# praeclarum/SdfKit

Measured on AMD Instinct MI355X. Metric: Mvoxels/s, 512^3 sphere SDF sample->mesh, higher is better.
Workload: dtype f32 (sampling) / f64 (cell math)

## Files before the change

include/sdfkit_hip.h:

```cpp
#ifndef SDFKIT_HIP_H
#define SDFKIT_HIP_H
#include <stdint.h>
#ifdef __cplusplus
extern "C" {
#endif
#if defined(__GNUC__) || defined(__clang__)
#pragma GCC visibility push(default)
#endif

#define SDFK_ABI_VERSION 6

typedef enum sdfk_status {
    SDFK_OK = 0,
    SDFK_ERR_INVALID = 1,
    SDFK_ERR_NO_DEVICE = 2,
    SDFK_ERR_HIP = 3,
    SDFK_ERR_COMPILE = 4,
    SDFK_ERR_NOMEM = 5,
    SDFK_ERR_UNSUPPORTED = 6
} sdfk_status;

typedef enum sdfk_opcode {
    SDFK_OP_CONST = 0,
    SDFK_OP_X = 1, SDFK_OP_Y = 2, SDFK_OP_Z = 3,
    SDFK_OP_ADD = 4, SDFK_OP_SUB = 5, SDFK_OP_MUL = 6, SDFK_OP_DIV = 7,
    SDFK_OP_NEG = 8, SDFK_OP_ABS = 9, SDFK_OP_SQRT = 10, SDFK_OP_FLOOR = 11,
    SDFK_OP_MIN_SEL = 12,
    SDFK_OP_MAX_SEL = 13,
    SDFK_OP_MIN_IEEE = 14,
    SDFK_OP_MAX_IEEE = 15,
    SDFK_OP_SEL_LT = 16,
    SDFK_OP_VOXEL_NEAREST = 17,
    SDFK_OP_VOXEL_LINEAR = 18,
    SDFK_OP_SIN = 19, SDFK_OP_COS = 20, SDFK_OP_EXP = 21, SDFK_OP_LOG = 22,
    SDFK_OP_ATAN2 = 23
} sdfk_opcode;
#define SDFK_MAX_VOLUMES 8

typedef struct sdfk_op {
    int32_t opcode;
    int32_t a, b, c, d;
    float imm;
} sdfk_op;

typedef struct sdfk_program sdfk_program;
typedef struct sdfk_volume sdfk_volume;
typedef struct sdfk_mesh sdfk_mesh;
typedef struct sdfk_march_job sdfk_march_job;

int sdfk_abi_version(void);
int sdfk_init(int device);
void sdfk_shutdown(void);
int sdfk_set_stream(void* hip_stream);
int sdfk_synchronize(void);
int sdfk_lane_begin(int32_t lane, void* wait_hip_event);
int sdfk_lane_end(int32_t caller_stream_waits);
const char* sdfk_last_error(void);

typedef enum sdfk_option {
    SDFK_OPT_LANES = 1,
    SDFK_OPT_TOKENS = 2,
    SDFK_OPT_GRAPHS = 3,
    SDFK_OPT_COPY_MODE = 4,
    SDFK_OPT_CORNER_EVAL = 5,
    SDFK_OPT_VCOLOR_EVAL = 6,
    SDFK_OPT_DIST_EXCHANGE = 7,
    SDFK_OPT_DIST_LANES = 8,
    SDFK_OPT_HW_QUEUES = 9,
    SDFK_OPT_CODE_CACHE = 10,
    SDFK_OPT_PREFAULT_HUGE = 11,
    SDFK_OPT_DIST_INDEX16 = 12,
    SDFK_OPT_STREAM_PLACEMENT = 13,
    SDFK_OPT_IDLE_LANE = 14,
    SDFK_OPT_IDLE_PROGRAMS = 15,
    SDFK_OPT_ELIDE_VOLUME = 16,
    SDFK_OPT_COLOR_PASSES = 17,
    SDFK_OPT_COUNT_ = 18
} sdfk_option;
int sdfk_set_option(int32_t key, int64_t value);
int sdfk_get_option(int32_t key, int64_t* value);
int sdfk_set_cache_dir(const char* path);

int sdfk_program_create(const sdfk_op* ops, int32_t n_ops, const int32_t out_rgbw[4],
                        int32_t writes_color, sdfk_program** out);
int sdfk_program_check(const sdfk_op* ops, int32_t n_ops, const int32_t out_rgbw[4], int32_t writes_color);
int sdfk_program_create_bound(const sdfk_op* ops, int32_t n_ops, const int32_t out_rgbw[4], int32_t writes_color,
                              const sdfk_volume* const* volumes, int32_t n_volumes, sdfk_program** out);
int sdfk_program_check_bound(const sdfk_op* ops, int32_t n_ops, const int32_t out_rgbw[4], int32_t writes_color, int32_t n_volumes);
const char* sdfk_program_source(const sdfk_program* p);
int sdfk_jit_stats(int64_t* n_compiled, int64_t* n_cache_hits, double* compile_ms_total);
void sdfk_program_destroy(sdfk_program* p);

int sdfk_volume_create(int32_t nx, int32_t ny, int32_t nz, const float min[3], const float max[3],
                       int32_t with_colors, sdfk_volume** out);
int sdfk_volume_create_slab(int32_t nx, int32_t ny, int32_t nz_global, const float min[3],
                            const float max[3], int32_t z0, int32_t nz_local,
                            int32_t with_colors, sdfk_volume** out);
int sdfk_volume_upload(sdfk_volume* v, const float* values, const float* colors3);
int sdfk_volume_download(const sdfk_volume* v, float* values, float* colors3);
int sdfk_volume_device_ptrs(const sdfk_volume* v, void** values, void** colors3);
int sdfk_volume_row_pitch(const sdfk_volume* v, int32_t* pitch_voxels);
void sdfk_volume_free(sdfk_volume* v);

int sdfk_sample(const sdfk_program* p, sdfk_volume* v, int32_t clip_to_bounds);
int sdfk_volume_clip_to_bounds(sdfk_volume* v);

int sdfk_march(const sdfk_volume* v, float iso_value, int32_t step, sdfk_mesh** out);
int sdfk_march_host(const float* values, const float* colors3, int32_t nx, int32_t ny, int32_t nz,
                    const float min[3], const float max[3], float iso_value, int32_t step,
                    sdfk_mesh** out);
int sdfk_sample_march(const sdfk_program* p, const float min[3], const float max[3],
                      int32_t nx, int32_t ny, int32_t nz, int32_t clip_to_bounds,
                      float iso_value, int32_t step, sdfk_mesh** out);
int sdfk_graph_stats(int64_t* jobs, int64_t* launches, int64_t* device_bytes);

int sdfk_march_begin(const sdfk_volume* v, float iso_value, int32_t layer_begin, int32_t layer_end,
                     sdfk_march_job** job, int64_t* n_vertices, int64_t* n_indices);
int sdfk_march_finish(sdfk_march_job* job, int64_t vertex_base, sdfk_mesh** out);
void sdfk_march_job_free(sdfk_march_job* job);

int sdfk_march_slab(const sdfk_volume* v, float iso_value, int32_t layer_begin, int32_t layer_end,
                    int64_t vertex_base, sdfk_mesh** out);
int sdfk_sample_march_slab(const sdfk_program* p, sdfk_volume* slab, int32_t clip_to_bounds, float iso_value,
                           int32_t layer_begin, int32_t layer_end, int64_t vertex_base, sdfk_mesh** out);

#define SDFK_SLAB_HEADER_BYTES 64
int sdfk_mesh_pack(const sdfk_mesh* m, void* dst, int64_t capacity_bytes, int64_t* needed_bytes);
int sdfk_slab_enqueue(const sdfk_program* p, sdfk_volume* slab, int32_t clip_to_bounds, float iso_value,
                      int32_t layer_begin, int32_t layer_end, void* dst, int64_t capacity_bytes,
                      int32_t lane, void* wait_hip_event);
int sdfk_slabs_rebase(void* gathered, int32_t world, int64_t stride_bytes);
int sdfk_slabs_rebase_mirror(void* gathered, int32_t world, int64_t stride_bytes, void* headers_mirror);

#define SDFK_DIST_ID_BYTES 128
int sdfk_dist_unique_id(void* id_out );
int sdfk_dist_init(int32_t world, int32_t rank, const void* id );
typedef int (*sdfk_allgather_fn)(void* ctx, const void* send, void* recv, int64_t bytes_per_rank);
int sdfk_dist_init_host(int32_t world, int32_t rank, sdfk_allgather_fn allgather, void* ctx);
int sdfk_dist_info(int32_t* world, int32_t* rank, int32_t* backend);
void sdfk_dist_shutdown(void);
int sdfk_dist_slab(int32_t nz, int32_t world, int32_t rank, int32_t* layer_begin, int32_t* layer_end, int32_t* z0, int32_t* nz_local);

#if defined(__GNUC__) || defined(__clang__)
#pragma GCC visibility pop
#endif
typedef struct sdfk_dist_session sdfk_dist_session;
#if defined(__GNUC__) || defined(__clang__)
#pragma GCC visibility push(default)
#endif
int sdfk_dist_session_create(const sdfk_program* p, const float min[3], const float max[3], int32_t nx, int32_t ny, int32_t nz,
                             int32_t clip_to_bounds, float iso_value, int32_t depth, sdfk_dist_session** out);
int sdfk_dist_submit(sdfk_dist_session* s);
int sdfk_dist_collect(sdfk_dist_session* s, int64_t* n_vertices_mine, int64_t* n_indices_mine);
int sdfk_dist_counts(const sdfk_dist_session* s, int64_t* counts);
int sdfk_dist_mesh(sdfk_dist_session* s, sdfk_mesh** out);
int sdfk_dist_slab_mesh(sdfk_dist_session* s, sdfk_mesh** out);
int sdfk_dist_gathered(const sdfk_dist_session* s, void** device_ptr, int64_t* stride_bytes);
int sdfk_dist_stats(const sdfk_dist_session* s, int64_t stats[8]);
int sdfk_dist_tune(sdfk_dist_session* s, int32_t steps_per_mode, int64_t* ns_per_config);
int sdfk_dist_enqueue_only(sdfk_dist_session* s);
// ... 205 lines not shown
```

sdfkit_amd/_native.py:

```python
import ctypes as C
import os
import sys

from . import build as _build

_HERE = os.path.dirname(os.path.abspath(__file__))
_lib = None
_inited_device = None


class SdfKitNativeError(RuntimeError):
    def __init__(self, status, message):
        super().__init__(f"sdfkit_hip status {status}: {message}")
        self.status = status


class Op(C.Structure):
    _fields_ = [("opcode", C.c_int32), ("a", C.c_int32), ("b", C.c_int32), ("c", C.c_int32),
                ("d", C.c_int32), ("imm", C.c_float)]


_vp, _i32, _i64, _f = C.c_void_p, C.c_int32, C.c_int64, C.c_float
_fp, _vpp = C.POINTER(C.c_float), C.POINTER(C.c_void_p)
SIGNATURES = {
# ... 89 lines not shown
    "sdfk_points_search": (C.c_int, [_vp, _vp, _i64, _vp, _vp, _vp]),
    "sdfk_points_search_device": (C.c_int, [_vp, _vp, _i64, _vp, _vp, _vp]),
    "sdfk_points_stats": (C.c_int, [_vp, C.POINTER(_i64)]),
    "sdfk_points_knn": (C.c_int, [_vp, _vp, _i64, _i32, _f, _vp, _vp, _vp]),
    "sdfk_points_knn_device": (C.c_int, [_vp, _vp, _i64, _i32, _f, _vp, _vp, _vp]),
    "sdfk_points_radius_count": (C.c_int, [_vp, _vp, _i64, _f, _vp]),
    "sdfk_points_radius_count_device": (C.c_int, [_vp, _vp, _i64, _f, _vp]),
    "sdfk_points_radius_fill": (C.c_int, [_vp, _vp, _i64, _f, _vp, _vp, _vp]),
    "sdfk_points_radius_fill_device": (C.c_int, [_vp, _vp, _i64, _f, _vp, _vp, _vp]),
    "sdfk_points_normals": (C.c_int, [_vp, _i32, _f, _vp, _i64, _vp, _vp]),
    "sdfk_points_normals_device": (C.c_int, [_vp, _i32, _f, _vp, _i64, _vp, _vp]),
    "sdfk_points_to_volume": (C.c_int, [_vp, _vp, _vp, _i32, _f, C.POINTER(_i64)]),
    "sdfk_points_to_volume_device": (C.c_int, [_vp, _vp, _vp, _i32, _f, C.POINTER(_i64)]),
    "sdfk_points_orient_normals": (C.c_int, [_vp, _i32, _f, _i32, _vp, C.POINTER(_i64)]),
    "sdfk_points_orient_normals_device": (C.c_int, [_vp, _i32, _f, _i32, _vp, C.POINTER(_i64)]),
    "sdfk_points_voxel_downsample": (C.c_int, [_vp, _f, _vp, _vp, _vp, _vp, C.POINTER(_i64)]),
    "sdfk_points_voxel_downsample_device": (C.c_int, [_vp, _f, _vp, _vp, _vp, _vp, C.POINTER(_i64)]),
    "sdfk_points_outliers": (C.c_int, [_vp, _i32, _f, _f, _vp, _vp, _vp, _vp, C.POINTER(_i64), C.POINTER(_i64)]),
    "sdfk_points_outliers_device": (C.c_int, [_vp, _i32, _f, _f, _vp, _vp, _vp, _vp, C.POINTER(_i64), C.POINTER(_i64)]),
    "sdfk_points_blend_colors": (C.c_int, [_vp, _vp, _vp, _i64, _i32, _f, _vp, _vp]),
    "sdfk_points_blend_colors_device": (C.c_int, [_vp, _vp, _vp, _i64, _i32, _f, _vp, _vp]),
    "sdfk_points_to_volume_colors": (C.c_int, [_vp, _vp, _vp, _vp, _i32, _f, C.POINTER(_i64)]),
    "sdfk_points_to_volume_colors_device": (C.c_int, [_vp, _vp, _vp, _vp, _i32, _f, C.POINTER(_i64)]),
    "sdfk_points_voxel_downsample_colors": (C.c_int, [_vp, _f, _vp, _vp, _vp, _vp, _vp, _vp, C.POINTER(_i64)]),
    "sdfk_points_voxel_downsample_colors_device": (C.c_int, [_vp, _f, _vp, _vp, _vp, _vp, _vp, _vp, C.POINTER(_i64)]),
    "sdfk_points_cluster": (C.c_int, [_vp, _f, _i32, _vp, _vp, _vp, _vp, C.POINTER(_i64), C.POINTER(_i64)]),
    "sdfk_points_cluster_device": (C.c_int, [_vp, _f, _i32, _vp, _vp, _vp, _vp, C.POINTER(_i64), C.POINTER(_i64)]),
    "sdfk_points_select": (C.c_int, [_vp, _vp, _vp, _i64, _vp, _vp, C.POINTER(_i64)]),
    "sdfk_points_select_device": (C.c_int, [_vp, _vp, _vp, _i64, _vp, _vp, C.POINTER(_i64)]),
    "sdfk_points_free": (None, [_vp]),
    "sdfk_trimesh_create": (C.c_int, [_vp, _i64, _vp, _i64, _vp, _vpp]),
    "sdfk_trimesh_create_device": (C.c_int, [_vp, _i64, _vp, _i64, _vp, _vpp]),
    "sdfk_trimesh_closest": (C.c_int, [_vp, _vp, _i64, _vp, _vp, _vp]),
    "sdfk_trimesh_closest_device": (C.c_int, [_vp, _vp, _i64, _vp, _vp, _vp]),
    "sdfk_trimesh_to_volume": (C.c_int, [_vp, _vp, C.c_float]),
    "sdfk_trimesh_stats": (C.c_int, [_vp, C.POINTER(_i64)]),
    "sdfk_trimesh_sample": (C.c_int, [_vp, _i64, C.c_uint64, _i32, _vp, _vp, _vp, _vp, _vp, C.POINTER(_i64)]),
    "sdfk_trimesh_sample_device": (C.c_int, [_vp, _i64, C.c_uint64, _i32, _vp, _vp, _vp, _vp, _vp, C.POINTER(_i64)]),
    "sdfk_trimesh_components": (C.c_int, [_vp, _vp, _vp, C.POINTER(_i64), C.POINTER(_i64)]),
    "sdfk_trimesh_components_device": (C.c_int, [_vp, _vp, _vp, C.POINTER(_i64), C.POINTER(_i64)]),
    "sdfk_trimesh_topology": (C.c_int, [_vp, C.POINTER(_i64), _vp, _i64]),
    "sdfk_trimesh_topology_device": (C.c_int, [_vp, C.POINTER(_i64), _vp, _i64]),
    "sdfk_trimesh_select": (C.c_int, [_vp, _vp, _vp, _vp, _vp, _vp, _vp, C.POINTER(_i64), C.POINTER(_i64)]),
    "sdfk_trimesh_select_device": (C.c_int, [_vp, _vp, _vp, _vp, _vp, _vp, _vp, C.POINTER(_i64), C.POINTER(_i64)]),
    "sdfk_trimesh_adjacency": (C.c_int, [_vp, _vp, _vp, _vp, C.POINTER(_i64)]),
    "sdfk_trimesh_adjacency_device": (C.c_int, [_vp, _vp, _vp, _vp, C.POINTER(_i64)]),
    "sdfk_trimesh_smooth": (C.c_int, [_vp, _i32, C.c_float, C.c_float, _i32, _vp]),
    "sdfk_trimesh_smooth_device": (C.c_int, [_vp, _i32, C.c_float, C.c_float, _i32, _vp]),
    "sdfk_trimesh_vertex_normals": (C.c_int, [_vp, _vp, _i32, _vp]),
    "sdfk_trimesh_vertex_normals_device": (C.c_int, [_vp, _vp, _i32, _vp]),
    "sdfk_trimesh_weld": (C.c_int, [_vp, C.c_float, _i32, _vp, _vp, _vp, _vp, _vp, _vp, C.POINTER(_i64), C.POINTER(_i64), C.POINTER(_i64)]),
    "sdfk_trimesh_weld_device": (C.c_int, [_vp, C.c_float, _i32, _vp, _vp, _vp, _vp, _vp, _vp, C.POINTER(_i64), C.POINTER(_i64), C.POINTER(_i64)]),
    "sdfk_trimesh_simplify": (C.c_int, [_vp, C.c_float, _i32, _i32, _vp, _vp, _vp, _vp, _vp, _vp, C.POINTER(_i64), C.POINTER(_i64), C.POINTER(_i64)]),
    "sdfk_trimesh_simplify_device": (C.c_int, [_vp, C.c_float, _i32, _i32, _vp, _vp, _vp, _vp, _vp, _vp, C.POINTER(_i64), C.POINTER(_i64), C.POINTER(_i64)]),
    "sdfk_trimesh_raycast": (C.c_int, [_vp, _vp, _vp, _i64, C.c_float, C.c_float, _i32, _vp, _vp, _vp]),
    "sdfk_trimesh_raycast_device": (C.c_int, [_vp, _vp, _vp, _i64, C.c_float, C.c_float, _i32, _vp, _vp, _vp]),
    "sdfk_trimesh_render": (C.c_int, [_vp, _i32, _i32, _fp, _fp, C.c_float, C.c_float, _vp, _vp, _vp]),
    "sdfk_trimesh_render_device": (C.c_int, [_vp, _i32, _i32, _fp, _fp, C.c_float, C.c_float, _vp, _vp, _vp]),
    "sdfk_trimesh_free": (None, [_vp]),
    "sdfk_volume_redistance": (C.c_int, [_vp, _vp, C.c_float, C.c_float, C.POINTER(_i64)]),
    "sdfk_icp_register": (C.c_int, [_vp, _vp, _vp, _i64, _fp, C.POINTER(_i32)]),
    "sdfk_icp_register_device": (C.c_int, [_vp, _vp, _vp, _i64, _fp, C.POINTER(_i32)]),
    "sdfk_icp_register_plane": (C.c_int, [_vp, _vp, _vp, _vp, _i64, _fp, C.POINTER(_i32), C.POINTER(_i64)]),
    "sdfk_icp_register_plane_device": (C.c_int, [_vp, _vp, _vp, _vp, _i64, _fp, C.POINTER(_i32), C.POINTER(_i64)]),
    "sdfk_profile_count": (C.c_int, []),
    "sdfk_profile_get": (C.c_int, [_i32, C.POINTER(C.c_char_p), C.POINTER(C.c_double), C.POINTER(_i64)]),
}


class IcpParams(C.Structure):
    _fields_ = [("max_iterations", C.c_int32), ("good_correspondence_distance", C.c_float),
                ("converged_max_translation", C.c_float), ("converged_max_rotation", C.c_float)]


ALLGATHER_FN = C.CFUNCTYPE(C.c_int, C.c_void_p, C.c_void_p, C.c_void_p, C.c_int64)

OK, ERR_INVALID, ERR_NO_DEVICE, ERR_HIP, ERR_COMPILE, ERR_NOMEM, ERR_UNSUPPORTED = 0, 1, 2, 3, 4, 5, 6

OPT_LANES, OPT_TOKENS, OPT_GRAPHS, OPT_COPY_MODE, OPT_CORNER_EVAL, OPT_VCOLOR_EVAL = 1, 2, 3, 4, 5, 6
OPT_DIST_EXCHANGE, OPT_DIST_LANES, OPT_HW_QUEUES, OPT_CODE_CACHE, OPT_PREFAULT_HUGE, OPT_DIST_INDEX16, OPT_STREAM_PLACEMENT, OPT_IDLE_LANE = 7, 8, 9, 10, 11, 12, 13, 14
OPT_IDLE_PROGRAMS = 15
OPT_ELIDE_VOLUME = 16
OPT_COLOR_PASSES = 17


def library_path():
    return os.environ.get("SDFKIT_HIP_LIBRARY") or os.path.join(_HERE, "libsdfkit_hip.so")


def lib():
    global _lib
    if _lib is None:
        path = library_path()
        if not os.environ.get("SDFKIT_HIP_LIBRARY") and (not os.path.exists(path) or _build.needs_build()):
            try:
                _build.build()
            except Exception as e:
                what = "is missing" if not os.path.exists(path) else "is older than its sources"
                raise RuntimeError(f"libsdfkit_hip.so {what} and could not be built with hipcc: {e}") from e
        if "torch" not in sys.modules and os.environ.get("SDFKIT_NO_TORCH_PRELOAD") != "1":
            try:
                import torch
            except Exception:
                pass
        L = C.CDLL(path)
        for name, (res, args) in SIGNATURES.items():
            fn = getattr(L, name)
            fn.restype = res
            fn.argtypes = args
        _lib = L
    return _lib


def check(status):
    if status != 0:
        raise SdfKitNativeError(status, lib().sdfk_last_error().decode("utf-8", "replace"))


def init(device=None):
    global _inited_device
    if device is None:
        device = int(os.environ.get("LOCAL_RANK", "0"))
    if _inited_device is None:
        check(lib().sdfk_init(device))
        _inited_device = device
    elif _inited_device != device:
        raise RuntimeError(f"sdfkit_hip already initialised on device {_inited_device}")
    return _inited_device


def bind_torch_stream(device=None):
    import torch
    s = torch.cuda.current_stream(device)
    if s.cuda_stream == 0:
        s = torch.cuda.Stream(device)
        torch.cuda.set_stream(s)
    check(lib().sdfk_set_stream(C.c_void_p(s.cuda_stream)))
    return s


class _PinnedBlock:

    def __init__(self, nbytes):
        p = C.c_void_p()
        check(lib().sdfk_host_alloc(int(nbytes), C.byref(p)))
        self.ptr, self.nbytes = p.value, int(nbytes)

    @property
    def __array_interface__(self):
        return {"shape": (self.nbytes,), "typestr": "|u1", "data": (self.ptr, False), "version": 3}

    def __del__(self):
        try:
            if self.ptr and _lib is not None and _inited_device is not None:
                _lib.sdfk_host_free(C.c_void_p(self.ptr))
        except Exception:
            pass
        self.ptr = 0


def pinned_empty(shape, dtype):
    import numpy as np
    dt = np.dtype(dtype)
    n = int(np.prod(shape)) * dt.itemsize
    if n == 0 or os.environ.get("SDFK_PINNED_ARRAYS") == "0":
        return np.empty(shape, dt)
# ... 55 lines not shown
```

sdfkit_amd/build.py:

```python
import os
import re
import subprocess
import sys
from concurrent.futures import ThreadPoolExecutor

HERE = os.path.dirname(os.path.abspath(__file__))
CSRC = os.path.join(HERE, "csrc")
OBJ = os.path.join(CSRC, "_obj")
LIB = os.path.join(HERE, "libsdfkit_hip.so")
SOURCES = ["lib_context.hip", "lib_jit.hip", "lib_volume.hip", "lib_march.hip", "lib_mesh.hip", "lib_dist.hip", "mc_kernels.hip", "lib_points.hip",
           "lib_trimesh.hip", "lib_redistance.hip", "lib_points_knn.hip", "lib_pointcloud.hip", "lib_orient.hip", "lib_points_filter.hip", "lib_trimesh_topology.hip",
           "lib_trimesh_smooth.hip", "lib_trimesh_weld.hip", "lib_points_cluster.hip", "lib_trimesh_simplify.hip", "lib_trimesh_ray.hip"]
HEADERS = ["lib_internal.h", "device_stage.h", "points_grid.h", "points_set.h", "points_knn.h", "points_walk.h", "points_normals.h", "points_orient.h", "points_filter.h", "points_color.h", "points_cluster.h", "device_forest.h", "icp_solve.h", "trimesh_sdf.h", "trimesh_sample.h", "trimesh_handle.h", "trimesh_topology.h", "trimesh_adjacency.h", "trimesh_weld.h", "trimesh_simplify.h", "trimesh_ray.h", "device_sort.h", "redistance.h", "device_scan.h", "device_reduce.h", "mc_kernels.h", "mc_device.h", "mc_decide.h", "mc_params.h", "mc_luts.h", "sample_codegen.h", "vol_pyramid.h", "mathops.h", "dist_rccl.h", "node_local.h",
           "slab_protocol.h", os.path.join("..", "..", "include", "sdfkit_hip.h")]
DEPS = ["exports.map"] + SOURCES + HEADERS
CFLAGS = ["--offload-arch=gfx950", "-O3", "-std=c++17", "-ffp-contract=off", "-fPIC", "-fno-fast-math", "-fvisibility=hidden", "-Wall",
          "-Wno-unused-function"]
EXTRA = os.environ.get("SDFKIT_HIP_CFLAGS", "").split()


def needs_build():
    if not os.path.exists(LIB):
        return True
    t = os.path.getmtime(LIB)
    return any(os.path.getmtime(os.path.join(CSRC, d)) > t for d in DEPS)


def _includes(path, seen):
    if path in seen or not os.path.exists(path):
        return
    seen.add(path)
    with open(path) as f:
        for m in re.finditer(r'^\s*#include\s+"([^"]+)"', f.read(), re.M):
            _includes(os.path.normpath(os.path.join(os.path.dirname(path), m.group(1))), seen)


def _object_for(src, hipcc, verbose, out_dir=None, extra=()):
    out_dir = out_dir or OBJ
    os.makedirs(out_dir, exist_ok=True)
    s = os.path.join(CSRC, src)
    o = os.path.join(out_dir, src.replace(".hip", ".o"))
    deps = set()
    _includes(s, deps)
    if not extra and os.path.exists(o) and all(os.path.getmtime(d) <= os.path.getmtime(o) for d in deps) and \
            os.path.getmtime(os.path.abspath(__file__)) <= os.path.getmtime(o):
        return o
    cmd = [hipcc] + CFLAGS + list(extra) + ["-c", s, "-o", o]
    if verbose:
        print(" ".join(cmd), file=sys.stderr)
    subprocess.check_call(cmd)
    return o


def build(force=False, verbose=False, out=None, extra=()):
    target = out or LIB
    extra = list(extra) + EXTRA
    if not out and not force and not needs_build():
        return LIB
    import fcntl
    with open(target + ".lock", "w") as lock:
        fcntl.flock(lock, fcntl.LOCK_EX)
        if not out and not force and not needs_build():
            return LIB
        hipcc = os.environ.get("HIPCC", "/opt/rocm/bin/hipcc")
        obj_dir = OBJ if not extra else os.path.join(OBJ, "variant_" + re.sub(r"\W+", "_", os.path.basename(target)))
        with ThreadPoolExecutor(max_workers=min(len(SOURCES), os.cpu_count() or 4)) as ex:
            objs = list(ex.map(lambda s: _object_for(s, hipcc, verbose, obj_dir, extra), SOURCES))
        tmp = f"{target}.tmp.{os.getpid()}"
        cmd = [hipcc, "--offload-arch=gfx950", "-shared", "-fPIC", "-Wl,--version-script=" + os.path.join(CSRC, "exports.map"), "-o", tmp] + objs + \
              ["-lhiprtc", "-ldl"]
        if verbose:
            print(" ".join(cmd), file=sys.stderr)
        try:
            subprocess.check_call(cmd)
            os.replace(tmp, target)
        finally:
            if os.path.exists(tmp):
                os.remove(tmp)
    return target


if __name__ == "__main__":
    args = [a for a in sys.argv[1:] if a != "--force"]
    if len(args) >= 1:
        build(force=True, verbose=True, out=os.path.abspath(args[0]), extra=args[1:])
    else:
        build(force="--force" in sys.argv, verbose=True)
```

sdfkit_amd/csrc/lib_context.hip:

```cpp
#include "lib_internal.h"

thread_local std::string t_err;
Config g_cfg;
DeviceState g_state0;
std::atomic<DeviceState*> g_default_state{&g_state0};
std::mutex g_registry_mu;
std::atomic<int> g_contexts_up{0};
std::vector<DeviceState*> g_states{&g_state0};
thread_local DeviceState* t_state = nullptr;
HostArena g_arena;
HostPool g_pool;
std::recursive_mutex g_pool_mu;

int fail(int code, const char* fmt, ...)
{
    char buf[1024];
    va_list ap;
    va_start(ap, fmt);
    vsnprintf(buf, sizeof buf, fmt, ap);
    va_end(ap);
    t_err = buf;
    return code;
}

// ... 358 lines not shown
            g_copy_stats[0] = (int64_t)total;
            g_copy_stats[1] = since(tp0);
            for (auto& p : pieces) { prefault_start(p.dst, p.bytes); g_pool.wait(); }
            g_copy_stats[2] = since(tp0);
            g_copy_stats[4] = 0;
            const int nt = g_pool.size() + 1;
            for (size_t k = 0; k < chunks.size() && e == hipSuccess; k++) {
                const auto tw = std::chrono::steady_clock::now();
                e = hipEventSynchronize(ev[k % kStageSlots]);
                g_copy_stats[4] += since(tw);
                if (e != hipSuccess) break;
                const Chunk c = chunks[k];
                const char* slot = (const char*)g.stage + (k % kStageSlots) * kStageChunk;
                const size_t per = (c.bytes + nt - 1) / nt;
                g_pool.start(nt, [=](int t) {
                    const size_t a = std::min((size_t)t * per, c.bytes), b = std::min(a + per, c.bytes);
                    if (b > a) memcpy(c.dst + a, slot + a, b - a);
                });
                g_pool.wait();
                if (issued < chunks.size()) e = issue(issued++);
            }
        }
        g_copy_stats[3] = since(tp0);
        if (e != hipSuccess) (void)hipStreamSynchronize(g.stream);
        for (auto& x : ev) g.prof_event_pool.push_back(x);
        if (e != hipSuccess) return fail(SDFK_ERR_HIP, "device-to-host copy: %s", hipGetErrorString(e));
        return SDFK_OK;
    }
    size_t k0 = 0;
    while (k0 < pieces.size() && pieces[k0].bytes == 0) k0++;
    prefault_start(pieces[k0].dst, pieces[k0].bytes);
    g_pool.wait();
    for (size_t k = k0; k < pieces.size(); k++) {
        size_t kn = k + 1;
        while (kn < pieces.size() && pieces[kn].bytes == 0) kn++;
        const bool more = kn < pieces.size();
        if (more) prefault_start(pieces[kn].dst, pieces[kn].bytes);
        hipError_t e = hipSuccess;
        if (pieces[k].bytes) {
            e = hipMemcpyAsync(pieces[k].dst, pieces[k].src, pieces[k].bytes, hipMemcpyDeviceToHost, g.stream);
            if (e == hipSuccess) e = hipStreamSynchronize(g.stream);
        }
        if (more) g_pool.wait();
        if (e != hipSuccess) return fail(SDFK_ERR_HIP, "device-to-host copy: %s", hipGetErrorString(e));
        k = kn - 1;
    }
    return SDFK_OK;
}


extern "C" int sdfk_abi_version(void) { return SDFK_ABI_VERSION; }

extern "C" const char* sdfk_last_error(void) { return t_err.c_str(); }

void config_from_env_once();
void config_from_env()
{
    static std::once_flag once;
    std::call_once(once, config_from_env_once);
}
void config_from_env_once()
{
    g_cfg.loaded = true;
    auto geti = [](const char* name, int dflt) { const char* e = getenv(name); return e && *e ? atoi(e) : dflt; };
    auto gets = [](const char* name) { const char* e = getenv(name); return std::string(e ? e : ""); };
    auto ranged = [&](const char* name, int dflt, int lo, int hi) { const int v = geti(name, dflt); return v >= lo && v <= hi ? v : dflt; };
    g_cfg.lanes = ranged("SDFK_LANES", 3, 0, Context::NSIDE);
    g_cfg.tokens = ranged("SDFK_TOKENS", -1, -1, 3);
    g_cfg.graphs = ranged("SDFK_GRAPHS", 1, 0, 2);
    g_cfg.copy_mode = ranged("SDFK_COPY_MODE", 1, 0, 2);
    g_cfg.copy_threads = ranged("SDFK_COPY_THREADS", 0, 0, 256);
    g_cfg.corner_eval = geti("SDFK_NO_CORNER_EVAL", 0) ? 0 : 1;
    g_cfg.vcolor_eval = geti("SDFK_NO_VCOLOR_EVAL", 0) ? 0 : 1;
    g_cfg.dist_exchange = ranged("SDFK_DIST_EXCHANGE", 0, 0, 3);
    g_cfg.dist_lanes = ranged("SDFK_DIST_LANES", 3, 0, 3);
    g_cfg.dist_index16 = geti("SDFK_DIST_INDEX16", 0) ? 1 : 0;
    g_cfg.code_cache = geti("SDFK_NO_CACHE", 0) ? 0 : 1;
    g_cfg.idle_programs = ranged("SDFK_IDLE_PROGRAMS", 32, 0, 1024);
    g_cfg.elide_volume = ranged("SDFK_ELIDE_VOLUME", 2, 0, 2);
    g_cfg.color_passes = ranged("SDFK_COLOR_PASSES", 0, 0, 2);
    g_cfg.prefault_huge = geti("SDFK_PREFAULT_HUGE", 0) ? 1 : 0;
    g_cfg.place_streams = geti("SDFK_STREAM_PLACEMENT", 1) ? 1 : 0;
    g_cfg.idle_lane = geti("SDFK_IDLE_LANE", 1) ? 1 : 0;
    g_cfg.sample_mode = geti("SDFK_SAMPLE_MODE", -1);
    g_cfg.hw_queues = geti("GPU_MAX_HW_QUEUES", 0);
    g_cfg.env_cache_dir = gets("SDFK_CACHE_DIR");
    g_cfg.env_xdg = gets("XDG_CACHE_HOME");
    g_cfg.env_home = gets("HOME");
    g_cfg.jit_flags = gets("SDFK_JIT_FLAGS");
    g_cfg.dump_source = gets("SDFK_DUMP_SOURCE");
    g_cfg.rccl_lib = gets("SDFK_RCCL_LIB");
}


int context_init(int device)
{
    std::lock_guard<std::recursive_mutex> lk(g_mu);
    if (g.inited) return SDFK_OK;
    int n = 0;
    hipError_t e = hipGetDeviceCount(&n);
    if (e != hipSuccess || n <= 0) return fail(SDFK_ERR_NO_DEVICE, "no HIP device: %s", hipGetErrorString(e));
    if (device < 0 || device >= n) return fail(SDFK_ERR_INVALID, "device %d out of range (%d devices)", device, n);
    HIPCHK(hipSetDevice(device));
    hipDeviceProp_t prop;
    HIPCHK(hipGetDeviceProperties(&prop, device));
    if (strncmp(prop.gcnArchName, "gfx950", 6) != 0)
        return fail(SDFK_ERR_NO_DEVICE, "device %d is %s; this library is built for gfx950 (MI355X) only", device, prop.gcnArchName);
    HIPCHK(hipStreamCreateWithFlags(&g.own_stream, hipStreamNonBlocking));
    g.user_stream = g.stream = g.own_stream;
    g.lanes[0].stream = g.own_stream;
    place_streams();
    for (int k = 1; k <= 3 && k <= Context::NSIDE; k++) (void)lane_stream(k);
    g.cur_lane = 0;
    HIPCHK(hipHostMalloc((void**)&g.slots, sizeof(Context::HostSlot) * Context::NSLOTS, hipHostMallocMapped));
    HIPCHK(hipHostGetDevicePointer((void**)&g.slots_dev, g.slots, 0));
    memset(g.slots, 0, sizeof(Context::HostSlot) * Context::NSLOTS);
    g.device = device;
    t_bound_device = device;
    g.inited = true;
    g_contexts_up.fetch_add(1);
    return SDFK_OK;
}

DeviceState* context_claim(int device, bool listed)
{
    std::lock_guard<std::mutex> rl(g_registry_mu);
    DeviceState* st = nullptr;
    if (listed)
        for (DeviceState* q : g_states)
            if (q->listed && q->claimed_device == device) st = q;
    DeviceState* const dflt = g_default_state.load(std::memory_order_relaxed);
    if (!st)
        for (DeviceState* q : g_states)
            if (q->claimed_device < 0 && (listed || q != dflt)) { st = q; break; }
    if (!st) {
        st = new DeviceState();
        g_states.push_back(st);
    }
    st->claimed_device = device;
    st->listed = listed;
    if (listed && (dflt->claimed_device < 0 || !dflt->listed)) g_default_state.store(st, std::memory_order_release);
    return st;
}

void context_unclaim(DeviceState* st)
{
    std::lock_guard<std::mutex> rl(g_registry_mu);
    st->claimed_device = -1;
    st->listed = true;
    if (g_default_state.load(std::memory_order_relaxed) == st)
        for (DeviceState* q : g_states)
            if (q->listed && q->claimed_device >= 0) { g_default_state.store(q, std::memory_order_release); break; }
}


extern "C" int sdfk_init(int device)
{
    config_from_env();
    if (device < 0) return fail(SDFK_ERR_INVALID, "device %d out of range", device);
    DeviceState* prev = t_state;
    DeviceState* st = context_claim(device, true);
    t_state = st;
    const int r = context_init(device);
    if (r) {
        bool inited;
        { std::lock_guard<std::recursive_mutex> lk(st->mu); inited = st->ctx.inited; }
        if (!inited) context_unclaim(st);
        t_state = prev;
    }
    return r;
}

extern "C" void sdfk_shutdown(void)
{
    std::lock_guard<std::recursive_mutex> lk(g_mu);
    bind_thread();
    if (!g.inited) return;
    while (!g.pending.empty()) (void)mesh_resolve(g.pending.front());
    graph_jobs_destroy_all();
    codes_drop_idle();
    if (dist_active()) dist_release();
    (void)hipStreamSynchronize(g.stream);
    prof_drain();
    for (auto e : g.prof_event_pool) (void)hipEventDestroy(e);
    g.prof_event_pool.clear();
    sync_all_lanes();
    for (auto& t : g.tokens) {
        for (auto& e : t.ring) { if (e) (void)hipEventDestroy(e); e = nullptr; }
        t.last = nullptr; t.last_lane = -1; t.next = 0;
    }
    for (auto& lane : g.lanes) {
        for (auto& kv : lane.free_blocks) (void)hipFree(kv.second);
        lane.free_blocks.clear();
        lane.clean_cull_headers.clear();
    }
    for (auto& kv : g.live_blocks) (void)hipFree(kv.first);
    g.live_blocks.clear();
    for (int k = 1; k <= Context::NSIDE; k++) {
        if (g.lane_done[k]) (void)hipEventDestroy(g.lane_done[k]);
        g.lane_done[k] = nullptr;
        bool pooled = false;
        for (const auto& q : g.pool) pooled = pooled || q.s == g.lanes[k].stream;
        if (g.lanes[k].stream && !pooled) (void)hipStreamDestroy(g.lanes[k].stream);
        g.lanes[k].stream = nullptr;
    }
    for (auto& q : g.pool) (void)hipStreamDestroy(q.s);
    g.pool.clear();
    g.foreign_cls.clear();
    g.placed = false;
    g.cls_lane0 = -1;
    g.n_classes = 0;
    if (g.spin_sink) (void)hipFree(g.spin_sink);
    g.spin_sink = nullptr;
    g.cur_lane = 0;
    g.lanes[0].stream = nullptr;
    for (auto& st : g.slot_state) {
        if (st.dropped) (void)hipEventDestroy(st.dropped);
        st = Context::SlotState();
    }
    if (g.stage) (void)hipHostFree(g.stage);
    g.stage = nullptr;
    g.stage_bytes = 0;
    {
        bool last = true;
        {
            std::lock_guard<std::mutex> rl(g_registry_mu);
            for (DeviceState* q : g_states) last = last && (q == &cur_state() || q->claimed_device < 0);
        }
        if (last) {
            std::lock_guard<std::mutex> al(g_arena.mu);
            for (auto& kv : g_arena.free_blocks) (void)hipHostFree(kv.second);
            g_arena.free_blocks.clear();
            g_arena.live.clear();
        }
    }
    if (g.slots) (void)hipHostFree(g.slots);
    g.slots = nullptr;
    g.slots_dev = nullptr;
    g.hints.clear();
    if (g.own_stream) (void)hipStreamDestroy(g.own_stream);
    g.own_stream = nullptr;
    g.stream = g.user_stream = nullptr;
    g.inited = false;
    g_contexts_up.fetch_sub(1);
    g.device = -1;
    context_unclaim(&cur_state());
}

extern "C" int sdfk_set_stream(void* hip_stream)
{
    std::lock_guard<std::recursive_mutex> lk(g_mu);
    if (int r = require_init()) return r;
    HIPCHK(hipStreamSynchronize(g.stream));
    g.user_stream = hip_stream ? (hipStream_t)hip_stream : g.own_stream;
    g.lanes[0].stream = g.user_stream;
    replace_lane0(g.user_stream);
    g.stream = g.lanes[g.cur_lane].stream;
    return SDFK_OK;
}

extern "C" int sdfk_lane_begin(int32_t lane, void* wait_hip_event)
{
    std::lock_guard<std::recursive_mutex> lk(g_mu);
    if (int r = require_init()) return r;
    if (lane < 1 || lane > Context::NSIDE) return fail(SDFK_ERR_INVALID, "sdfk_lane_begin: lane %d out of range 1..%d", lane, Context::NSIDE);
    if (g.cur_lane != 0) return fail(SDFK_ERR_INVALID, "sdfk_lane_begin: already inside a lane section");
    hipStream_t ls = lane_stream(lane);
    if (wait_hip_event) HIPCHK(hipStreamWaitEvent(ls, (hipEvent_t)wait_hip_event, 0));
    g.cur_lane = lane;
    g.stream = ls;
    return SDFK_OK;
}

extern "C" int sdfk_lane_end(int32_t caller_stream_waits)
{
    std::lock_guard<std::recursive_mutex> lk(g_mu);
    if (int r = require_init()) return r;
    if (g.cur_lane == 0) return fail(SDFK_ERR_INVALID, "sdfk_lane_end: not inside a lane section");
    const int lane = g.cur_lane;
    g.cur_lane = 0;
    g.stream = g.lanes[0].stream;
    if (caller_stream_waits) {
        hipEvent_t ev = g.lane_done[lane];
        if (!ev) {
            HIPCHK(hipEventCreateWithFlags(&ev, hipEventDisableTiming));
            g.lane_done[lane] = ev;
        }
        hipError_t e = hipEventRecord(ev, lane_stream(lane));
        if (e == hipSuccess) e = hipStreamWaitEvent(g.lanes[0].stream, ev, 0);
        if (e != hipSuccess) return fail(SDFK_ERR_HIP, "sdfk_lane_end: %s", hipGetErrorString(e));
    }
    return SDFK_OK;
}

extern "C" int sdfk_synchronize(void)
{
    std::lock_guard<std::recursive_mutex> lk(g_mu);
    if (int r = require_init()) return r;
    HIPCHK(hipStreamSynchronize(g.stream));
    sync_all_lanes();
    for (auto& st : g.slot_state) st.drop_pending = false;
    return SDFK_OK;
}

void codes_trim();
extern "C" int sdfk_set_option(int32_t key, int64_t value)
{
    std::lock_guard<std::recursive_mutex> lk(g_mu);
    config_from_env();
    auto in = [&](int64_t lo, int64_t hi) { return value >= lo && value <= hi; };
    switch (key) {
    case SDFK_OPT_LANES: if (!in(0, Context::NSIDE)) break; g_cfg.lanes = (int)value; return SDFK_OK;
    case SDFK_OPT_TOKENS: if (!in(-1, 3)) break; g_cfg.tokens = (int)value; return SDFK_OK;
    case SDFK_OPT_GRAPHS: if (!in(0, 2)) break; g_cfg.graphs = (int)value; return SDFK_OK;
    case SDFK_OPT_COPY_MODE: if (!in(0, 2)) break; g_cfg.copy_mode = (int)value; return SDFK_OK;
    case SDFK_OPT_CORNER_EVAL: if (!in(0, 1)) break; g_cfg.corner_eval = (int)value; return SDFK_OK;
    case SDFK_OPT_VCOLOR_EVAL: if (!in(0, 1)) break; g_cfg.vcolor_eval = (int)value; return SDFK_OK;
    case SDFK_OPT_DIST_EXCHANGE: if (!in(0, 3)) break; g_cfg.dist_exchange = (int)value; return SDFK_OK;
    case SDFK_OPT_DIST_LANES: if (!in(0, 3)) break; g_cfg.dist_lanes = (int)value; return SDFK_OK;
    case SDFK_OPT_DIST_INDEX16: if (!in(0, 1)) break; g_cfg.dist_index16 = (int)value; return SDFK_OK;
    case SDFK_OPT_STREAM_PLACEMENT: if (!in(0, 1)) break; g_cfg.place_streams = (int)value; return SDFK_OK;
    case SDFK_OPT_IDLE_LANE: if (!in(0, 1)) break; g_cfg.idle_lane = (int)value; return SDFK_OK;
    case SDFK_OPT_CODE_CACHE: if (!in(0, 1)) break; g_cfg.code_cache = (int)value; return SDFK_OK;
    case SDFK_OPT_IDLE_PROGRAMS: if (!in(0, 1024)) break; g_cfg.idle_programs = (int)value; codes_trim(); return SDFK_OK;
    case SDFK_OPT_ELIDE_VOLUME: if (!in(0, 2)) break; g_cfg.elide_volume = (int)value; return SDFK_OK;
    case SDFK_OPT_COLOR_PASSES: if (!in(0, 2)) break; g_cfg.color_passes = (int)value; return SDFK_OK;
    case SDFK_OPT_PREFAULT_HUGE: if (!in(0, 1)) break; g_cfg.prefault_huge = (int)value; return SDFK_OK;
    case SDFK_OPT_HW_QUEUES: return fail(SDFK_ERR_INVALID, "SDFK_OPT_HW_QUEUES is read-only");
    default: return fail(SDFK_ERR_INVALID, "sdfk_set_option: unknown option %d", key);
    }
    return fail(SDFK_ERR_INVALID, "sdfk_set_option(%d): value %lld out of range", key, (long long)value);
}

extern "C" int sdfk_get_option(int32_t key, int64_t* value)
{
    std::lock_guard<std::recursive_mutex> lk(g_mu);
    if (!value) return fail(SDFK_ERR_INVALID, "sdfk_get_option: null argument");
    config_from_env();
    switch (key) {
    case SDFK_OPT_LANES: *value = g_cfg.lanes; break;
    case SDFK_OPT_TOKENS: *value = g_cfg.tokens; break;
    case SDFK_OPT_GRAPHS: *value = g_cfg.graphs; break;
    case SDFK_OPT_COPY_MODE: *value = g_cfg.copy_mode; break;
    case SDFK_OPT_CORNER_EVAL: *value = g_cfg.corner_eval; break;
    case SDFK_OPT_VCOLOR_EVAL: *value = g_cfg.vcolor_eval; break;
    case SDFK_OPT_DIST_EXCHANGE: *value = g_cfg.dist_exchange; break;
    case SDFK_OPT_DIST_LANES: *value = g_cfg.dist_lanes; break;
    case SDFK_OPT_DIST_INDEX16: *value = g_cfg.dist_index16; break;
    case SDFK_OPT_STREAM_PLACEMENT: *value = g_cfg.place_streams; break;
    case SDFK_OPT_IDLE_LANE: *value = g_cfg.idle_lane; break;
    case SDFK_OPT_CODE_CACHE: *value = g_cfg.code_cache; break;
    case SDFK_OPT_IDLE_PROGRAMS: *value = g_cfg.idle_programs; break;
    case SDFK_OPT_ELIDE_VOLUME: *value = g_cfg.elide_volume; break;
    case SDFK_OPT_COLOR_PASSES: *value = g_cfg.color_passes; break;
    case SDFK_OPT_PREFAULT_HUGE: *value = g_cfg.prefault_huge; break;
    case SDFK_OPT_HW_QUEUES: *value = g_cfg.hw_queues; break;
    default: return fail(SDFK_ERR_INVALID, "sdfk_get_option: unknown option %d", key);
    }
    return SDFK_OK;
}

extern "C" int sdfk_set_cache_dir(const char* path)
{
    std::lock_guard<std::recursive_mutex> lk(g_mu);
    config_from_env();
    g_cfg.cache_dir_set = path != nullptr;
    g_cfg.cache_dir = path ? path : "";
    return SDFK_OK;
}

extern "C" int sdfk_host_alloc(int64_t n_bytes, void** out)
{
    if (!out || n_bytes < 0) return fail(SDFK_ERR_INVALID, "sdfk_host_alloc: bad argument");
    *out = nullptr;
    if (g_contexts_up.load() <= 0) {
        std::lock_guard<std::recursive_mutex> lk(g_mu);
        if (int r = require_init()) return r;
    }
    const size_t c = size_class((size_t)std::max<int64_t>(n_bytes, 1));
    std::lock_guard<std::mutex> al(g_arena.mu);
    auto it = g_arena.free_blocks.upper_bound(c);
    void* p = nullptr;
    if (it != g_arena.free_blocks.begin() && std::prev(it)->first == c) {
        --it;
        p = it->second;
        g_arena.free_blocks.erase(it);
    } else if (hipHostMalloc(&p, c, hipHostMallocPortable) != hipSuccess) {
        (void)hipGetLastError();
        for (auto& kv : g_arena.free_blocks) (void)hipHostFree(kv.second);
        g_arena.free_blocks.clear();
        if (hipHostMalloc(&p, c, hipHostMallocPortable) != hipSuccess) { (void)hipGetLastError(); return fail(SDFK_ERR_NOMEM, "hipHostMalloc(%zu) failed", c); }
    }
    g_arena.live[p] = c;
    *out = p;
    return SDFK_OK;
}

extern "C" void sdfk_host_free(void* p)
{
    if (!p) return;
    std::lock_guard<std::mutex> al(g_arena.mu);
    auto it = g_arena.live.find(p);
    if (it == g_arena.live.end()) return;
    g_arena.free_blocks.emplace(it->second, p);
    g_arena.live.erase(it);
}

extern "C" int sdfk_stream_placement(int32_t out[8])
{
    std::lock_guard<std::recursive_mutex> lk(g_mu);
    if (!out) return fail(SDFK_ERR_INVALID, "sdfk_stream_placement: null argument");
    if (int r = require_init()) return r;
    out[0] = g.placed && !g.pool.empty() ? 1 : 0;
    out[1] = g.n_classes;
    out[2] = g.cls_lane0;
    for (int k = 1; k <= 4; k++) {
        out[2 + k] = -1;
        for (const auto& q : g.pool)
            if (k <= Context::NSIDE && q.s == g.lanes[k].stream) out[2 + k] = q.cls;
    }
    out[7] = -1;
    for (const auto& q : g.pool)
        if (q.user == 100) out[7] = q.cls;
    return SDFK_OK;
}

extern "C" int sdfk_copy_stats(int64_t stats[5])
{
    std::lock_guard<std::recursive_mutex> lk(g_mu);
    if (!stats) return fail(SDFK_ERR_INVALID, "sdfk_copy_stats: null argument");
    memcpy(stats, g_copy_stats, sizeof g_copy_stats);
    return SDFK_OK;
}
// ... 53 lines not shown
```

sdfkit_amd/csrc/lib_internal.h:

```cpp
#pragma once
#include <hip/hip_runtime.h>
#include <hip/hiprtc.h>

#include <fcntl.h>
#include <sys/mman.h>
#include <sys/stat.h>
#include <unistd.h>

#include <algorithm>
#include <atomic>
#include <cerrno>
#include <chrono>
#include <cmath>
#include <condition_variable>
#include <cstdarg>
#include <cstdio>
#include <cstring>
#include <deque>
#include <functional>
#include <map>
#include <memory>
#include <mutex>
#include <string>
#include <thread>
#include <unordered_map>
#include <vector>

#include <rccl/rccl.h>

#include "../../include/sdfkit_hip.h"
#include "mc_kernels.h"
#include "sample_codegen.h"

using namespace sdfk;

extern thread_local std::string t_err;
static constexpr int kSampleRpw = 2;


struct Config {
    bool loaded = false;
    int lanes = 3;
    int tokens = -1;
    int graphs = 1;
    int copy_mode = 1;
    int corner_eval = 1;
    int vcolor_eval = 1;
    int dist_exchange = 0;
    int dist_lanes = 3;
    int dist_index16 = 0;
    int code_cache = 1;
    int idle_programs = 32;
    int color_passes = 0;
    int elide_volume = 2;
    int prefault_huge = 0;
    int place_streams = 1;
    int idle_lane = 1;
    int copy_threads = 0;
    int sample_mode = -1;
    int hw_queues = 0;
    std::string cache_dir;
    bool cache_dir_set = false;
    std::string jit_flags;
    std::string dump_source;
    std::string env_cache_dir, env_xdg, env_home, rccl_lib;
};
extern Config g_cfg;

int fail(int code, const char* fmt, ...);
#define HIPCHK(expr)                                                                              \
    do {                                                                                          \
        hipError_t e_ = (expr);                                                                   \
        if (e_ != hipSuccess) return fail(SDFK_ERR_HIP, "%s: %s (%s:%d)", #expr, hipGetErrorString(e_), __FILE__, __LINE__); \
    } while (0)

struct sdfk_mesh;
struct sdfk_volume;
struct ProgCode;



struct ProfSpan { int name_id; hipEvent_t a, b; };

struct Context {
    bool inited = false;
    int device = -1;
    hipStream_t stream = nullptr;
    hipStream_t user_stream = nullptr;
    hipStream_t own_stream = nullptr;
    static constexpr int NSIDE = 4;
    struct Lane { hipStream_t stream = nullptr; std::multimap<size_t, void*> free_blocks; std::vector<uint32_t*> clean_cull_headers; };
    Lane lanes[1 + NSIDE];
    struct Placed { hipStream_t s; int cls; int user; };
    std::vector<Placed> pool;
    std::map<hipStream_t, int> foreign_cls;
    int cls_lane0 = -1, n_classes = 0;
    bool placed = false;
    int* spin_sink = nullptr;
    hipEvent_t lane_done[1 + NSIDE] = {};
    int cur_lane = 0;
    int side_lanes = 2;
    int next_side = 0;
    struct Token { hipEvent_t ring[8] = {}; int next = 0; hipEvent_t last = nullptr; int last_lane = -1; };
    Token tokens[2];
    int token_mask = 0;
    struct Block { size_t size; int lane; };
    std::map<void*, Block> live_blocks;
    bool prof_on = false;
    bool sampler_only = false;
    std::vector<std::string> prof_names;
    std::vector<double> prof_ms;
    std::vector<int64_t> prof_n;
    std::vector<ProfSpan> prof_pending;
    std::vector<hipEvent_t> prof_event_pool;
    struct HostSlot { McCounters c; float bounds[8]; };
    static constexpr int NSLOTS = 64;
    HostSlot* slots = nullptr;
    HostSlot* slots_dev = nullptr;
    int slot_next = 0;
    struct SlotState { bool busy = false; bool drop_pending = false; hipEvent_t dropped = nullptr; };
    SlotState slot_state[NSLOTS];
    void* stage = nullptr;
    size_t stage_bytes = 0;
    struct Hint { uint32_t n_active, nv, ni; };
    std::map<uint64_t, Hint> hints;
    std::deque<sdfk_mesh*> pending;
    static constexpr size_t MAX_PENDING = 6;
    std::vector<struct GraphJob*> graph_jobs;
    uint64_t graph_clock = 0;
    size_t graph_bytes = 0;
    int64_t graph_launches = 0;
    std::map<uint64_t, uint32_t> graph_sightings;
};

struct RcclApi {
    void* handle = nullptr;
    ncclResult_t (*GetUniqueId)(ncclUniqueId*) = nullptr;
    ncclResult_t (*CommInitRank)(ncclComm_t*, int, ncclUniqueId, int) = nullptr;
    ncclResult_t (*CommDestroy)(ncclComm_t) = nullptr;
    ncclResult_t (*AllGather)(const void*, void*, size_t, ncclDataType_t, ncclComm_t, hipStream_t) = nullptr;
    ncclResult_t (*Send)(const void*, size_t, ncclDataType_t, int, ncclComm_t, hipStream_t) = nullptr;
    ncclResult_t (*Recv)(void*, size_t, ncclDataType_t, int, ncclComm_t, hipStream_t) = nullptr;
    ncclResult_t (*GroupStart)() = nullptr;
    ncclResult_t (*GroupEnd)() = nullptr;
    const char* (*GetErrorString)(ncclResult_t) = nullptr;
};

struct DistContext {
    int backend = 0;
    int world = 1, rank = 0;
    RcclApi nccl;
    ncclComm_t comm = nullptr;
    hipStream_t stream = nullptr;
    bool stream_owned = false;
    sdfk_allgather_fn host_fn = nullptr;
    void* host_ctx = nullptr;
    int64_t* agree_dev = nullptr;
    int64_t* agree_host = nullptr;
    char* stage = nullptr;
    int64_t stage_stride = 0;
    int sessions = 0;
    int (*consensus_fn)(void* ctx, int mine) = nullptr;
    void* consensus_ctx = nullptr;
};

struct DeviceState {
    Context ctx;
    std::recursive_mutex mu;
    DistContext dist;
    std::unordered_map<std::string, ProgCode*> codes;
    uint64_t code_clock = 0;
    int graph_build_failures = 0;
    int claimed_device = -1;
    bool listed = true;
// ... 102 lines not shown
        if (threads.empty())
            for (int i = 0; i < size(); i++) threads.emplace_back([this] { worker(); });
        fn = std::move(f);
        ntasks = n;
        next = 0;
        generation++;
        cv_work.notify_all();
    }
    void wait()
    {
        std::unique_lock<std::mutex> lk(mu);
        while (next < ntasks) {
            const int t = next++;
            running++;
            lk.unlock();
            fn(t);
            lk.lock();
            running--;
        }
        cv_done.wait(lk, [&] { return running == 0; });
        ntasks = 0;
    }
    ~HostPool()
    {
        {
            std::unique_lock<std::mutex> lk(mu);
            stopping = true;
            cv_work.notify_all();
        }
        for (auto& t : threads) t.join();
    }
};

extern HostPool g_pool;
extern std::recursive_mutex g_pool_mu;

struct CopyPiece { const void* src; void* dst; size_t bytes; };

constexpr int kTwoPassMaxOps = 24;
constexpr size_t kTwoPassMinVoxels = size_t(1) << 21;
enum ProgKernel { PK_BITS = 0, PK_BITS_FLAT = 1, PK_SIGNS = 2, PK_BITS_CLIP = 3, PK_BITS_CLIP_FLAT = 4, PK_VCOLORS = 5, PK_CORNERS = 6, PK_RAYMARCH = 7,
                  PK_SIGNS_FLAT = 8, PK_CULL = 9, PK_EVAL_BLOCKS = 10, PK_POINTS = 11,
                  PK_BITS_NC = 12, PK_BITS_NC_FLAT = 13, PK_BITS_NC_CLIP = 14, PK_BITS_NC_CLIP_FLAT = 15, PK_COLORS = 16, PK_COUNT = 17 };
inline bool pk_is_sampler(int k) { return k <= PK_BITS_CLIP_FLAT || k == PK_SIGNS_FLAT || k == PK_CULL || k == PK_EVAL_BLOCKS || (k >= PK_BITS_NC && k <= PK_BITS_NC_CLIP_FLAT); }

struct ProgCode {
    std::string source;
    std::vector<hipModule_t> modules;
    hipFunction_t fn[PK_COUNT] = {};
    int refs = 0;
    uint64_t last_use = 0;
};

struct sdfk_program {
    ProgCode* code = nullptr;
    std::vector<float> params;
    int writes_color = 0;
    int n_ops = 0;
    int refs = 1;
    bool orphaned = false;
    bool no_elide = false;
    void* vol_mem = nullptr;
    DeviceState* owner = nullptr;
    std::vector<uint64_t> kbuf;
    void* kargs() const { return kbuf.empty() ? (void*)const_cast<float*>(params.data()) : (void*)const_cast<uint64_t*>(kbuf.data()); }
};

struct sdfk_volume {
    DeviceState* owner = &cur_state();
    int nx = 0, ny = 0, nz = 0;
    int nz_global = 0, z0 = 0;
    float gmin[3], gmax[3];
    float* values = nullptr;
    float* colors = nullptr;
    bool elided = false, elided_colors = false;
    uint32_t* cull_list = nullptr;
    uint32_t* cull_header = nullptr;
    mutable bool cull_header_clean = false;
    int cull_header_lane = 0;
    uint64_t* bits = nullptr;
    uint8_t* bits8 = nullptr;
    float bits_iso = 0.0f;
    bool bits_valid = false;
    sdfk_program* sampled_by = nullptr;
    SampleArgs sampled_args;
    int pitch() const { return (nz + 3) & ~3; }
    size_t nvox() const { return (size_t)nx * ny * nz; }
    size_t nalloc() const { return (size_t)nx * ny * pitch(); }
    int nxw() const { return (nx + 63) / 64; }
    int nx8() const { return (nx + 7) / 8; }
    int pitch8() const { return (nz + 3) & ~3; }
    size_t nbitwords() const { return (size_t)nz * ny * nxw() + 8; }
};

struct sdfk_mesh {
    DeviceState* owner = &cur_state();
    int64_t nv = 0, ni = 0;
    float* vertices = nullptr;
    float* colors = nullptr;
    float* normals = nullptr;
    int32_t* triangles = nullptr;
    float* bounds = nullptr;
    float h_min[3] = {0, 0, 0}, h_max[3] = {0, 0, 0};
    bool bounds_valid = false;
    int64_t n_active = 0, n_case13 = 0;
    size_t cap_v = 0, cap_i = 0;
    sdfk_march_job* pending = nullptr;
    hipEvent_t done = nullptr;
    const sdfk_volume* src = nullptr;
    bool owns_src = false;
    float iso = 0.0f;
    int step = 1, layer_begin = 0, layer_end = 0;
    int64_t vertex_base = 0;
    uint64_t key = 0;
    int status = 0;
    std::string error;
    bool has_colors = true;
    bool colors_valid = true;
    bool external = false;
    struct GraphJob* graph_job = nullptr;
    bool borrowed = false;
    void* slab_header = nullptr;
    int lane = 0;
    bool used_on_main = false;
};

struct sdfk_march_job {
    McParams P;
    McCounters c;
    std::vector<void*> owned;
    sdfk_volume* sub = nullptr;
    int gnx, gny, gnz;
    float gmin[3], gmax[3];
    bool finished = false;
    bool empty = false;
    bool have_bits = false;
    uint8_t* bits8 = nullptr;
    sdfk_program* eval_prog = nullptr;
    SampleArgs eval_args;
    bool colors_elided = false;
    int slot = -1;
    int lane = 0;
    bool* cull_clean = nullptr;
    float* bounds_partial = nullptr;
    int bounds_blocks = 0;
    uint2* vdesc = nullptr;
    size_t vdesc_cap = 0;
    size_t rec_first = 0;
};


int mesh_resolve(sdfk_mesh* m);
void graph_job_retire(sdfk_mesh* m, bool too_small);
void graph_jobs_destroy_all();
void graph_jobs_forget_volume(const sdfk_volume* v);
void graph_jobs_forget_program(const sdfk_program* p);
void dist_release();
bool dist_active();
void resolve_dependents(const sdfk_volume* v);
void free_mesh_buffers(sdfk_mesh* m);
void drop_source(sdfk_mesh* m);
void job_release(sdfk_march_job* j, bool kernels_may_be_queued = false);
void program_release(sdfk_program* p);
void volume_values_changed(sdfk_volume* v);
void codes_drop_idle();



struct GraphJob;
struct PostCompact { char* out; int64_t out_capacity; unsigned long long* ticket; };

void codes_trim();
size_t size_class(size_t n);
int dev_alloc(void** p, size_t n);
void dev_free(void* p);
hipStream_t lane_stream(int k);
void phase_token_wait(int kind);
void phase_token_pass(int kind);
void sync_all_lanes();
double chains_us(hipStream_t a, hipStream_t b);
int stream_class(hipStream_t s, const std::vector<hipStream_t>& reps, double serial_us);
void assign_placed_streams();
void place_streams();
void replace_lane0(hipStream_t s0);
hipStream_t placed_exchange_stream();
int prof_name_id(const char* name);
hipEvent_t prof_event();
void prof_drain();
int require_init();
void bind_thread();
int grid_for(size_t work_items, int per_block = 256, int max_blocks = 256 * 8);
void prefault_start(void* p, size_t n);
int stage_reserve();
int copy_to_host(const std::vector<CopyPiece>& pieces, const std::function<void()>& beside = nullptr);
void config_from_env();
void config_from_env_once();
int context_init(int device);
DeviceState* context_claim(int device, bool listed);
void context_unclaim(DeviceState* st);
uint64_t fnv1a64(const std::string& s, uint64_t h);
std::string cache_dir();
bool cache_load(const std::string& path, const std::string& key, std::vector<char>& code);
void cache_store(const std::string& path, const std::string& key, const std::vector<char>& code);
int compile_source(const std::string& src, unsigned mask, std::vector<char>& code, bool use_cache, bool* from_cache = nullptr,
                          bool refresh = false);
void code_unload(ProgCode* c);
ProgCode* code_acquire(std::string&& src);
void code_release(ProgCode* c);
int generate_source(const sdfk_op* ops, int32_t n_ops, const int32_t out_rgbw[4], int32_t writes_color, std::string& src,
                           std::vector<float>* params = nullptr, int n_volumes = 0);
int program_fn(const sdfk_program* cp, int k, hipFunction_t* fn);
int job_volume_create(const sdfk_program* p, int nx, int ny, int nz, const float mn[3], const float mx[3], float iso, sdfk_volume** out);
int volume_materialize(sdfk_volume* v);
dim3 transpose_grid(int nz, int ny, int nxw);
dim3 flat_grid(size_t plane, int nx8);
void grid_constants(const sdfk_volume* v, float d[3], float m[3], float* outside);
int sample_impl(const sdfk_program* p, sdfk_volume* v, int32_t clip_to_bounds, float iso_hint);
int acquire_slot();
int alloc_records(sdfk_march_job* j, size_t c);
// ... 31 lines not shown
```

sdfkit_amd/csrc/lib_march.hip:

```cpp
#include "lib_internal.h"



template <typename T>
int job_alloc(sdfk_march_job* j, T** p, size_t count)
{
    void* q = nullptr;
    if (int r = dev_alloc(&q, count * sizeof(T))) return r;
    j->owned.push_back(q);
    *p = (T*)q;
    return SDFK_OK;
}

int acquire_slot()
{
    for (int pass = 0; pass < 2; pass++) {
        int oldest = -1;
        for (int i = 0; i < Context::NSLOTS; i++) {
            const int s = (g.slot_next + i) % Context::NSLOTS;
            Context::SlotState& st = g.slot_state[s];
            if (st.busy) continue;
            if (st.drop_pending) {
                if (hipEventQuery(st.dropped) != hipSuccess) { if (oldest < 0) oldest = s; continue; }
                st.drop_pending = false;
            }
            st.busy = true;
            g.slot_next = (s + 1) % Context::NSLOTS;
            memset(&g.slots[s], 0, sizeof(Context::HostSlot));
            return s;
        }
        if (oldest < 0) break;
        (void)hipEventSynchronize(g.slot_state[oldest].dropped);
    }
    return -1;
}

void job_release(sdfk_march_job* j, bool kernels_may_be_queued)
{
    if (j->slot >= 0) {
        Context::SlotState& st = g.slot_state[j->slot];
        st.busy = false;
        st.drop_pending = false;
        if (kernels_may_be_queued) {
            hipError_t e = hipSuccess;
            if (!st.dropped) e = hipEventCreateWithFlags(&st.dropped, hipEventDisableTiming);
            if (e == hipSuccess) e = hipEventRecord(st.dropped, lane_stream(j->lane));
            if (e == hipSuccess) st.drop_pending = true;
            else (void)hipStreamSynchronize(lane_stream(j->lane));
        }
        j->slot = -1;
    }
    for (void* p : j->owned) dev_free(p);
    j->owned.clear();
    if (j->eval_prog) program_release(j->eval_prog);
    j->eval_prog = nullptr;
    if (j->sub) {
        dev_free(j->sub->values);
        dev_free(j->sub->colors);
        delete j->sub;
        j->sub = nullptr;
    }
}

#ifndef SDFK_COMPACT_MASKS
#define SDFK_COMPACT_MASKS 1
#endif
#ifndef SDFK_COMPACT_STRIDED
#define SDFK_COMPACT_STRIDED 1
#endif

int alloc_records(sdfk_march_job* j, size_t c)
{
    McParams& P = j->P;
    for (size_t k = j->rec_first; k < j->owned.size(); k++) dev_free(j->owned[k]);
    j->owned.resize(j->rec_first);
    j->bounds_partial = nullptr;
    j->vdesc = nullptr;
    j->vdesc_cap = 0;
    int rr = 0;
    rr = rr ? rr : job_alloc(j, &P.rec_xy, c);
    rr = rr ? rr : job_alloc(j, &P.rec_z, c);
    rr = rr ? rr : job_alloc(j, &P.rec_info, c);
    rr = rr ? rr : job_alloc(j, &P.rec_own, c);
    rr = rr ? rr : job_alloc(j, &P.rec_pre, c);
    rr = rr ? rr : job_alloc(j, &P.rec_corners, c * 8);
    rr = rr ? rr : job_alloc(j, &P.rec_vid, (c / MC_CHUNK + 1) * (size_t)MC_VSTRIDE);
    rr = rr ? rr : job_alloc(j, &P.chunkslots, c / MC_CHUNK + 2);
    rr = rr ? rr : job_alloc(j, &P.chunktot, c / MC_CHUNK + 2);
    rr = rr ? rr : job_alloc(j, &P.chunkpre, c / MC_CHUNK + 2);
    rr = rr ? rr : job_alloc(j, &P.chunkdead, c / MC_CHUNK + 2);
    rr = rr ? rr : job_alloc(j, &P.chunkwin, c / MC_CHUNK + 2);
    rr = rr ? rr : job_alloc(j, &P.chunkwin2, c / MC_CHUNK + 2);
    P.cap_active = (uint32_t)c;
    P.chunkscan = c / MC_CHUNK + 1 > MC_SCAN_CHUNKS ? 1 : 0;
    return rr;
}

int launch_classify(sdfk_march_job* j, bool publish)
{
    McParams& P = j->P;
    if (!j->have_bits) {
        uint64_t* bits = const_cast<uint64_t*>(P.bits);
        ProfScope ps("k_signbits");
        const int nx8 = (P.nx + 7) / 8, pitch8 = P.nzp;
        if ((P.nz % 256) != 0 || P.ny > 65535 || nx8 > 65535)
            hipLaunchKernelGGL(k_signbits8<true>, flat_grid((size_t)P.ny * pitch8, nx8), dim3(256), 0, g.stream,
                               P.values, j->bits8, P.nx, P.ny, P.nz, nx8, pitch8, P.iso);
        else
            hipLaunchKernelGGL(k_signbits8<false>, dim3((P.nz + 255) / 256, P.ny, nx8), dim3(256), 0, g.stream, P.values, j->bits8, P.nx, P.ny,
                               P.nz, nx8, pitch8, P.iso);
        hipLaunchKernelGGL(k_bits_transpose, transpose_grid(P.nz, P.ny, P.nxw), dim3(256), 0, g.stream, j->bits8, bits,
                           nx8, P.ny, P.nz, P.nxw, pitch8);
        HIPCHK(hipGetLastError());
        j->have_bits = true;
    }
    {
        ProfScope ps("k_compact");
        const int nwg = ((P.lay_list_end - P.lay_count_begin + K2_LPB - 1) / K2_LPB) * P.bpl;
        hipLaunchKernelGGL(k_compact<false>, dim3(nwg), dim3(256), 0, g.stream, P);
        HIPCHK(hipGetLastError());
        if (P.zero_cull && j->cull_clean && nwg > 0) *j->cull_clean = true;
        if (P.blockpre) hipLaunchKernelGGL(k_blockscan, dim3(1), dim3(1024), 0, g.stream, P);
        if (SDFK_COMPACT_STRIDED && K2_LPB == 1)
            if (P.segmask) hipLaunchKernelGGL(k_compact_write<true>, dim3((P.lay_list_end - P.lay_count_begin) * P.bpl), dim3(256), 0, g.stream, P);
            else hipLaunchKernelGGL(k_compact_write<false>, dim3((P.lay_list_end - P.lay_count_begin) * P.bpl), dim3(256), 0, g.stream, P);
        else
            hipLaunchKernelGGL(k_compact<true>, dim3(nwg), dim3(256), 0, g.stream, P);
        HIPCHK(hipGetLastError());
    }
    const int nchunks = (int)((P.cap_active + MC_CHUNK - 1u) / MC_CHUNK);
    if (j->eval_prog) {
        hipFunction_t fn_corners = nullptr;
        if (int r = program_fn(j->eval_prog, PK_CORNERS, &fn_corners)) return r;
        ProfScope ps("sdfk_corners_eval");
        const unsigned* n_active = &P.counters->n_active;
        void* params[] = {&j->eval_args, &P.rec_xy, &P.rec_z, &P.rec_corners, &n_active, &P.cap_active, &P.xbits, j->eval_prog->kargs()};
        HIPCHK(hipModuleLaunchKernel(fn_corners, (unsigned)std::min(nchunks, 256 * 8), 1, 1, 256, 1, 1, 0,
                                     g.stream, params, nullptr));
    } else {
        ProfScope ps("k_gather_corners");
        hipLaunchKernelGGL(k_gather_corners, dim3(std::min(nchunks, 256 * 8)), dim3(256), 0, g.stream, P);
        HIPCHK(hipGetLastError());
    }
    {
        ProfScope ps("k_resolve");
        constexpr int cap = 256 * 12;
        hipLaunchKernelGGL(k_resolve, dim3(std::min(nchunks, cap)), dim3(256), 0, g.stream, P);
        if (P.chunkscan) hipLaunchKernelGGL(k_chunkscan, dim3(1), dim3(1024), 0, g.stream, P);
        if (publish) hipLaunchKernelGGL(k_publish, dim3(1), dim3(256), 0, g.stream, P);
        HIPCHK(hipGetLastError());
    }
    return SDFK_OK;
}

int wait_counters(sdfk_march_job* j)
{
    HIPCHK(hipStreamSynchronize(g.stream));
    j->c = g.slots[j->slot].c;
    return SDFK_OK;
}

int setup_job(const sdfk_volume* v, float iso, int step, int layer_begin, int layer_end, size_t cap_records,
              sdfk_march_job** out)
{
    *out = nullptr;
    if (step < 1) return fail(SDFK_ERR_INVALID, "step must be >= 1");
    const bool slab = (v->z0 != 0 || v->nz != v->nz_global);
    if (step != 1 && (slab || layer_begin != 0)) return fail(SDFK_ERR_UNSUPPORTED, "slab meshing supports step == 1 only");
    sdfk_march_job* j = new sdfk_march_job();
    j->gnx = v->nx; j->gny = v->ny; j->gnz = v->nz_global;
    memcpy(j->gmin, v->gmin, sizeof j->gmin);
    memcpy(j->gmax, v->gmax, sizeof j->gmax);
    j->lane = g.cur_lane;
    j->slot = acquire_slot();
    if (j->slot < 0) { delete j; return fail(SDFK_ERR_NOMEM, "more than %d marching-cubes jobs are alive", Context::NSLOTS); }
    const sdfk_volume* w = v;
    if (step > 1) {
        sdfk_volume* s = new sdfk_volume(*v);
        s->nx = (v->nx - 1) / step + 1; s->ny = (v->ny - 1) / step + 1; s->nz = (v->nz - 1) / step + 1;
        s->nz_global = s->nz;
        s->values = nullptr; s->colors = nullptr; s->bits = nullptr; s->bits8 = nullptr; s->bits_valid = false; s->sampled_by = nullptr;
        j->sub = s;
        int r = dev_alloc((void**)&s->values, s->nalloc() * sizeof(float));
        if (!r && v->colors) r = dev_alloc((void**)&s->colors, s->nalloc() * 3 * sizeof(float));
        if (r) { job_release(j); delete j; return r; }
        ProfScope ps("k_subsample");
        hipLaunchKernelGGL(k_subsample, dim3(grid_for(s->nvox())), dim3(256), 0, g.stream, v->values, v->colors,
                           s->values, s->colors, v->nx, v->ny, v->pitch(), s->nx, s->ny, s->nz, s->pitch(), step);
        w = s;
        layer_end = s->nz - 1;
    }
    McParams& P = j->P;
    memset(&P, 0, sizeof P);
    P.values = w->values; P.colors = w->colors;
    j->colors_elided = w->elided && w->elided_colors;
    if (w->elided && w->cull_header && w->cull_header_lane == g.cur_lane) { P.zero_cull = w->cull_header; j->cull_clean = &w->cull_header_clean; }
    if (w->elided && (step != 1 || !w->sampled_by || !g_cfg.corner_eval || (w->elided_colors && !g_cfg.vcolor_eval) || !w->bits_valid || w->bits_iso != iso)) {
        job_release(j); delete j;
        return fail(SDFK_ERR_INVALID, "internal: a volume without storage can only be meshed by the program that sampled it (step 1, same iso)");
    }
    P.nx = w->nx; P.ny = w->ny; P.nz = w->nz;
    P.nzp = w->pitch();
    {
        auto bits = [](int n) { int b = 0; while ((1 << b) < n) b++; return b; };
        const int bx = bits(w->nx), by = bits(w->ny);
        P.xbits = by > 16 ? 32 - by : std::max(16, bx);
        P.xmask = P.xbits >= 32 ? 0xffffffffu : ((1u << P.xbits) - 1u);
    }
    P.ncx = w->nx - 1; P.ncy = w->ny - 1; P.ncz = w->nz - 1;
    P.nxw = (w->nx + 63) / 64;
    P.z0 = w->z0;
    P.iso = iso;
    P.step = step;
    const int ncz_global = w->nz_global - 1;
    if (layer_begin < 0 || layer_end > std::max(ncz_global, 0) || layer_begin > layer_end) {
        job_release(j); delete j;
        return fail(SDFK_ERR_INVALID, "layer range [%d,%d) outside [0,%d)", layer_begin, layer_end, ncz_global);
    }
    P.lay_emit_begin = layer_begin - w->z0;
    P.lay_emit_end = layer_end - w->z0;
    P.lay_count_begin = layer_begin > 0 ? P.lay_emit_begin - 1 : P.lay_emit_begin;
    P.lay_list_end = std::min(P.lay_emit_end + 1, P.ncz);
    j->empty = (P.ncx <= 0 || P.ncy <= 0 || P.ncz <= 0 || layer_begin == layer_end);
    memset(&j->c, 0, sizeof j->c);
    if (j->empty) { *out = j; return SDFK_OK; }
    {
        const int need_lo = std::max(layer_begin - 2, 0), need_hi = std::min(layer_end + 2, w->nz_global);
        if (w->z0 > need_lo || w->z0 + w->nz < need_hi) {
            job_release(j); delete j;
            return fail(SDFK_ERR_INVALID, "slab planes [%d,%d) do not cover the context [%d,%d) of layers [%d,%d)",
                        w->z0, w->z0 + w->nz, need_lo, need_hi, layer_begin, layer_end);
        }
    }
    P.bpl = (int)(((size_t)P.ncy * P.nxw + 1023) / 1024);
    const size_t ncell = (size_t)P.ncx * P.ncy * P.ncz;
    if (cap_records == 0) cap_records = std::max<size_t>(ncell / 12, 1u << 16);
    cap_records = std::min(cap_records, ncell);
    int r = 0;
    if (step == 1 && v->sampled_by && g_cfg.corner_eval) {
        j->eval_prog = v->sampled_by;
        j->eval_prog->refs++;
        j->eval_args = v->sampled_args;
    }
    j->have_bits = (step == 1 && v->bits && v->bits_valid && v->bits_iso == iso);
    if (j->have_bits) P.bits = v->bits;
    else {
        uint64_t* bits = nullptr;
        r = r ? r : job_alloc(j, &bits, (size_t)P.nz * P.ny * P.nxw + 8);
        P.bits = bits;
        r = r ? r : job_alloc(j, &j->bits8, (size_t)P.ny * ((P.nx + 7) / 8) * ((P.nz + 3) & ~3) + 64);
    }
    r = r ? r : job_alloc(j, &P.blockcnt, (size_t)(P.lay_list_end - P.lay_count_begin) * P.bpl + 1);
    r = r ? r : job_alloc(j, &P.wavecnt, (size_t)(P.lay_list_end - P.lay_count_begin) * P.bpl * 4 + 4);
    P.segmask = nullptr;
    if (SDFK_COMPACT_STRIDED && K2_LPB == 1 && SDFK_COMPACT_MASKS)
        r = r ? r : job_alloc(j, &P.segmask, (size_t)(P.lay_list_end - P.lay_count_begin) * P.bpl * 1024 + 4);
    P.blockpre = nullptr;
    if ((P.lay_list_end - P.lay_count_begin) * P.bpl > MC_SCAN_BLOCKS && SDFK_COMPACT_STRIDED && K2_LPB == 1)
        r = r ? r : job_alloc(j, &P.blockpre, (size_t)(P.lay_list_end - P.lay_count_begin) * P.bpl + 1);
    r = r ? r : job_alloc(j, &P.rowstart, (size_t)(P.lay_list_end - P.lay_count_begin) * P.ncy + 2);
    r = r ? r : job_alloc(j, &P.counters, 1);
    P.host_counters = &g.slots_dev[j->slot].c;
    j->rec_first = j->owned.size();
    r = r ? r : alloc_records(j, cap_records);
    if (r) { job_release(j); delete j; return r; }
    *out = j;
    return SDFK_OK;
}

int alloc_mesh(sdfk_mesh** out, size_t cap_v, size_t cap_i)
{
    sdfk_mesh* m = new sdfk_mesh();
    int r = 0;
    r = r ? r : dev_alloc((void**)&m->vertices, std::max<size_t>(cap_v, 1) * 3 * sizeof(float));
    r = r ? r : dev_alloc((void**)&m->colors, std::max<size_t>(cap_v, 1) * 3 * sizeof(float));
    r = r ? r : dev_alloc((void**)&m->normals, std::max<size_t>(cap_v, 1) * 3 * sizeof(float));
    r = r ? r : dev_alloc((void**)&m->triangles, std::max<size_t>(cap_i, 1) * sizeof(int32_t));
    r = r ? r : dev_alloc((void**)&m->bounds, 8 * sizeof(float));
    if (r) { sdfk_mesh_free(m); return r; }
    m->lane = g.cur_lane;
    m->cap_v = cap_v; m->cap_i = cap_i;
    *out = m;
    return SDFK_OK;
}

int launch_emit(sdfk_march_job* j, sdfk_mesh* m, int64_t vertex_base)
{
    McMeshOut M;
    memset(&M, 0, sizeof M);
    M.vertices = m->vertices; M.colors = m->colors; M.normals = m->normals; M.triangles = m->triangles;
    m->has_colors = j->P.colors != nullptr || j->colors_elided;
    if (!m->has_colors) {
        M.colors = nullptr;
        m->colors_valid = false;
    }
    M.cap_vertices = (uint32_t)m->cap_v;
    M.cap_indices = m->cap_i;
    M.vertex_base = vertex_base;
    M.slab_header = m->slab_header;
    M.slab_vbytes = m->has_colors ? 36 : 24;
    const int nn[3] = {j->gnx, j->gny, j->gnz};
    for (int k = 0; k < 3; k++) {
        const float size = j->gmax[k] - j->gmin[k];
        const float sum = j->gmin[k] + j->gmax[k];
        const float center = sum * 0.5f;
        const float t1 = (float)(-(nn[k] - 1)) / 2.0f;
        M.sc[k] = size / (float)(nn[k] - 1);
        const float ts = t1 * M.sc[k];
        M.tr[k] = ts + center;
    }
    {
        const float yz = M.sc[1] * M.sc[2], xz = M.sc[0] * M.sc[2], xy = M.sc[0] * M.sc[1];
        const float det = M.sc[0] * yz;
        const float inv_det = 1.0f / det;
        M.inv[0] = yz * inv_det; M.inv[1] = xz * inv_det; M.inv[2] = xy * inv_det;
    }
#ifndef SDFK_KV_GRIDCAP
#define SDFK_KV_GRIDCAP (256 * 8)
#endif
    constexpr int vcap = SDFK_KV_GRIDCAP, tcap = 256 * 8;
    const int vgrid = grid_for(j->P.cap_active, (int)MC_CHUNK, vcap);
    if (!j->bounds_partial || j->bounds_blocks != vgrid) {
        if (int rr = job_alloc(j, &j->bounds_partial, (size_t)vgrid * 6)) return rr;
        j->bounds_blocks = vgrid;
    }
    M.bounds_partial = j->bounds_partial;
    M.bounds_blocks = vgrid;
    const bool no_vcol = !g_cfg.vcolor_eval;
    const bool vcol = j->eval_prog && j->eval_prog->writes_color && (j->P.colors || j->colors_elided) && M.colors && j->P.step == 1 && !no_vcol;
    if (vcol) {
        const size_t need = std::max<size_t>(m->cap_v, 1);
        if (!j->vdesc || j->vdesc_cap < need) {
            if (int rr = job_alloc(j, &j->vdesc, need)) return rr;
            j->vdesc_cap = need;
        }
        M.vdesc = j->vdesc;
// ... 713 lines not shown
    return SDFK_OK;
}

int slab_enqueue_impl(const sdfk_program* p, sdfk_volume* slab, int32_t clip_to_bounds, float iso_value, int32_t layer_begin,
                             int32_t layer_end, void* dst, int64_t capacity_bytes, int32_t lane, void* wait_hip_event, bool caller_stream_waits,
                             const PostCompact* pc)
{
    int r = lane > 0 ? sdfk_lane_begin(lane, wait_hip_event) : SDFK_OK;
    if (r) return r;
    sdfk_mesh* m = nullptr;
    r = require_init();
    if (!r && lane > 0 && graphs_enabled_slab((int64_t)slab->nx * slab->ny * slab->nz)) {
        bool handled = false;
        r = graph_slab_enqueue(p, slab, clip_to_bounds ? 1 : 0, iso_value, layer_begin, layer_end, dst, capacity_bytes, &handled, pc);
        if (handled || r) {
            const int r2 = sdfk_lane_end(caller_stream_waits ? 1 : 0);
            return r ? r : r2;
        }
    }
    if (!r) r = sample_impl(p, slab, clip_to_bounds, iso_value);
    if (!r) r = march_range(slab, iso_value, 1, layer_begin, layer_end, 0, &m, (char*)dst, capacity_bytes);
    if (!r && !(m->external && m->pending)) {
        int64_t need = 0;
        r = sdfk_mesh_pack(m, dst, capacity_bytes, &need);
    }
    if (m) sdfk_mesh_free(m);
    if (!r) r = launch_post_compact(pc, dst, capacity_bytes);
    if (lane > 0) {
        const int r2 = sdfk_lane_end(caller_stream_waits ? 1 : 0);
        if (!r) r = r2;
    }
    return r;
}

extern "C" int sdfk_slab_enqueue(const sdfk_program* p, sdfk_volume* slab, int32_t clip_to_bounds, float iso_value,
                                 int32_t layer_begin, int32_t layer_end, void* dst, int64_t capacity_bytes,
                                 int32_t lane, void* wait_hip_event)
{
    std::lock_guard<std::recursive_mutex> lk(g_mu);
    if (!p || !slab || !dst) return fail(SDFK_ERR_INVALID, "sdfk_slab_enqueue: null argument");
    if (capacity_bytes < SDFK_SLAB_HEADER_BYTES) return fail(SDFK_ERR_INVALID, "sdfk_slab_enqueue: capacity below the header size");
    return slab_enqueue_impl(p, slab, clip_to_bounds, iso_value, layer_begin, layer_end, dst, capacity_bytes, lane, wait_hip_event, true);
}

int slabs_rebase(void* gathered, int32_t world, int64_t stride_bytes, void* headers_mirror)
{
    std::lock_guard<std::recursive_mutex> lk(g_mu);
    if (!gathered || world < 1 || stride_bytes < SDFK_SLAB_HEADER_BYTES) return fail(SDFK_ERR_INVALID, "sdfk_slabs_rebase: bad argument");
    if (int r = require_init()) return r;
    if (world == 1 && !headers_mirror) return SDFK_OK;
    hipLaunchKernelGGL(k_slabs_rebase, dim3(64, world), dim3(256), 0, g.stream, (char*)gathered, (int)world, (int64_t)stride_bytes,
                       (SlabHeader*)headers_mirror, 0);
    HIPCHK(hipGetLastError());
    return SDFK_OK;
}

extern "C" int sdfk_slabs_rebase(void* gathered, int32_t world, int64_t stride_bytes)
{
    return slabs_rebase(gathered, world, stride_bytes, nullptr);
}

extern "C" int sdfk_slabs_rebase_mirror(void* gathered, int32_t world, int64_t stride_bytes, void* headers_mirror)
{
    if (!headers_mirror) return fail(SDFK_ERR_INVALID, "sdfk_slabs_rebase_mirror: null mirror");
    return slabs_rebase(gathered, world, stride_bytes, headers_mirror);
}

extern "C" int sdfk_march_host(const float* values, const float* colors3, int32_t nx, int32_t ny, int32_t nz,
                               const float min[3], const float max[3], float iso_value, int32_t step,
                               sdfk_mesh** out)
{
    std::lock_guard<std::recursive_mutex> lk(g_mu);
    if (!values || !out) return fail(SDFK_ERR_INVALID, "sdfk_march_host: null argument");
    sdfk_volume* v = nullptr;
    int r = sdfk_volume_create(nx, ny, nz, min, max, colors3 ? 1 : 0, &v);
    if (r) return r;
    r = sdfk_volume_upload(v, values, colors3);
    if (!r) r = sdfk_march(v, iso_value, step, out);
    if (!r && (*out)->pending && (*out)->src == v) (*out)->owns_src = true;
    else sdfk_volume_free(v);
    return r;
}

extern "C" int sdfk_sample_march(const sdfk_program* p, const float min[3], const float max[3],
                                 int32_t nx, int32_t ny, int32_t nz, int32_t clip_to_bounds,
                                 float iso_value, int32_t step, sdfk_mesh** out)
{
    std::lock_guard<std::recursive_mutex> lk(g_mu);
    if (!p || !out) return fail(SDFK_ERR_INVALID, "sdfk_sample_march: null argument");
    if (int r = require_init()) return r;
    int lane = g.cur_lane;
    g.side_lanes = std::max(0, std::min(Context::NSIDE, g_cfg.lanes));
    if (g.side_lanes == 1) g.side_lanes = 0;
    const bool chain_only = step == 1 && g_cfg.elide_volume && g_cfg.corner_eval && g_cfg.vcolor_eval && !p->no_elide && iso_value == iso_value &&
                            !g.sampler_only;
    if (g.side_lanes == 3 && g_cfg.idle_lane && Context::NSIDE >= 4 && g.cur_lane == 0 && g.placed && step == 1 &&
        (graphs_enabled((int64_t)nx * ny * nz) || chain_only)) {
        bool placed4 = false;
        for (const auto& q : g.pool) placed4 = placed4 || (q.user == 4 && q.s == g.lanes[4].stream);
        if (placed4) {
            if (hipStreamQuery(g.lanes[0].stream) == hipSuccess) g.side_lanes = 4;
            else (void)hipGetLastError();
        }
    }
    if (g.side_lanes > 0 && g.cur_lane == 0) {
        if (g.next_side >= g.side_lanes) g.next_side = 0;
        lane = 1 + g.next_side;
        g.next_side = (g.next_side + 1) % g.side_lanes;
    }
    LaneScope on_lane(lane);
    *out = nullptr;
    if (step == 1 && graphs_enabled((int64_t)nx * ny * nz)) {
        if (int r = graph_sample_march(p, min, max, nx, ny, nz, clip_to_bounds ? 1 : 0, iso_value, out)) return r;
        if (*out) return SDFK_OK;
    }
    sdfk_volume* v = nullptr;
    const bool elidable = step == 1 && !graphs_enabled((int64_t)nx * ny * nz);
    int r = elidable ? job_volume_create(p, nx, ny, nz, min, max, iso_value, &v) : sdfk_volume_create(nx, ny, nz, min, max, p->writes_color ? 1 : 0, &v);
    if (r) return r;
    r = require_init();
    {
        const int dflt = (int64_t)nx * ny * nz >= (int64_t(1) << 27) ? 1 : 0;
        g.token_mask = (lane > 0 && g.side_lanes > 1) ? (g_cfg.tokens >= 0 ? g_cfg.tokens : dflt) : 0;
    }
    if (!r) r = sample_impl(p, v, clip_to_bounds, step == 1 ? iso_value : 0.0f);
    if (!r) r = sdfk_march(v, iso_value, step, out);
    g.token_mask = 0;
    if (!r && (*out)->pending && (*out)->src == v) (*out)->owns_src = true;
    else sdfk_volume_free(v);
    return r;
}
```

sdfkit_amd/csrc/lib_volume.hip:

```cpp
#include "lib_internal.h"
#include "device_stage.h"

void volume_values_changed(sdfk_volume* v)
{
    v->bits_valid = false;
    if (v->sampled_by) program_release(v->sampled_by);
    v->sampled_by = nullptr;
}


extern "C" int sdfk_volume_create_slab(int32_t nx, int32_t ny, int32_t nz_global, const float min[3],
                                       const float max[3], int32_t z0, int32_t nz_local,
                                       int32_t with_colors, sdfk_volume** out)
{
    std::lock_guard<std::recursive_mutex> lk(g_mu);
    if (!out || !min || !max) return fail(SDFK_ERR_INVALID, "sdfk_volume_create: null argument");
    *out = nullptr;
    if (nx < 1 || ny < 1 || nz_global < 1 || nz_local < 1 || z0 < 0 || z0 + nz_local > nz_global)
        return fail(SDFK_ERR_INVALID, "sdfk_volume_create: bad dimensions %dx%dx%d (slab z0=%d nz=%d)", nx, ny, nz_global, z0, nz_local);
    if ((int64_t)nx * ny * nz_global >= (int64_t(1) << 31))
        return fail(SDFK_ERR_INVALID, "grid exceeds the reference's int32 linear index (Voxels.cs:82)");
    if ((int64_t)nx * ny * ((nz_local + 3) & ~3) >= (int64_t(1) << 31))
        return fail(SDFK_ERR_INVALID, "grid with rows padded to %d voxels exceeds 2^31 voxel slots", (nz_local + 3) & ~3);
    if (int r = require_init()) return r;
// ... 116 lines not shown
        if (colors3 && v->colors) {
            if (int r = dev_alloc((void**)&dense_c, v->nvox() * 3 * sizeof(float))) { dev_free(dense_v); return r; }
            hipLaunchKernelGGL(k_repitch<false>, dim3(grid_for(v->nvox() * 3)), dim3(256), 0, g.stream, v->colors, dense_c, rows, v->nz * 3, v->pitch() * 3);
        }
    }
    struct FreeTmp { float *a, *b; ~FreeTmp() { dev_free(a); dev_free(b); } } free_tmp{dense_v, dense_c};
    if (values) pieces.push_back({dense_v ? dense_v : v->values, values, v->nvox() * sizeof(float)});
    if (colors3 && v->colors) pieces.push_back({dense_c ? dense_c : v->colors, colors3, v->nvox() * 3 * sizeof(float)});
    if (colors3 && !v->colors) {
        std::lock_guard<std::recursive_mutex> pool_lk(g_pool_mu);
        const size_t nb = v->nvox() * 3 * sizeof(float), per = size_t(2) << 20;
        char* c = (char*)colors3;
        g_pool.start((int)((nb + per - 1) / per), [=](int t) { const size_t a = (size_t)t * per; memset(c + a, 0, std::min(per, nb - a)); });
        g_pool.wait();
    }
    return copy_to_host(pieces);
}

extern "C" int sdfk_volume_row_pitch(const sdfk_volume* v, int32_t* pitch_voxels)
{
    if (!v || !pitch_voxels) return fail(SDFK_ERR_INVALID, "sdfk_volume_row_pitch: null argument");
    *pitch_voxels = v->pitch();
    return SDFK_OK;
}

extern "C" int sdfk_volume_device_ptrs(const sdfk_volume* v, void** values, void** colors3)
{
    std::lock_guard<std::recursive_mutex> lk(g_mu);
    bind_thread();
    if (!v) return fail(SDFK_ERR_INVALID, "null volume");
    resolve_dependents(v);
    volume_values_changed(const_cast<sdfk_volume*>(v));
    if (values) *values = v->values;
    if (colors3) *colors3 = v->colors;
    return SDFK_OK;
}

dim3 transpose_grid(int nz, int ny, int nxw)
{
    const unsigned groups = (unsigned)((nxw + 7) / 8);
    return dim3((unsigned)((nz + 127) / 128) * (unsigned)ny, (groups + 65534u) / 65535u, std::min(groups, 65535u));
}
dim3 flat_grid(size_t plane, int nx8)
{
    return dim3((unsigned)((plane + 255) / 256), ((unsigned)nx8 + 65534u) / 65535u, std::min((unsigned)nx8, 65535u));
}

void grid_constants(const sdfk_volume* v, float d[3], float m[3], float* outside)
{
    const int n[3] = {v->nx, v->ny, v->nz_global};
    for (int k = 0; k < 3; k++) {
        d[k] = n[k] >= 1 ? (v->gmax[k] - v->gmin[k]) / (float)n[k] : 0.0f;
        const float h = 0.5f * d[k];
        m[k] = v->gmin[k] + h;
    }
    *outside = (v->gmax[0] - v->gmin[0]) / (float)v->nx;
}


int sample_impl(const sdfk_program* p, sdfk_volume* v, int32_t clip_to_bounds, float iso_hint)
{
    SampleArgs A;
    memset(&A, 0, sizeof A);
    float d[3], m[3], outside;
    grid_constants(v, d, m, &outside);
    A.values = v->values;
    A.colors = v->colors;
    A.mx = m[0]; A.my = m[1]; A.mz = m[2];
    A.dx = d[0]; A.dy = d[1]; A.dz = d[2];
    A.nx = v->nx; A.ny = v->ny; A.nz = v->nz;
    A.z0 = v->z0; A.nz_global = v->nz_global;
    A.clip = clip_to_bounds ? 1 : 0;
    A.outside = outside;
    resolve_dependents(v);
    volume_values_changed(v);
    auto sampled = [&]() {
        sdfk_program* q = const_cast<sdfk_program*>(p);
        q->refs++;
        v->sampled_by = q;
        v->sampled_args = A;
    };
    void* params[] = {&A, p->kargs()};
    {
        if (!v->bits) {
            if (int r = dev_alloc((void**)&v->bits, v->nbitwords() * sizeof(uint64_t))) return r;
        }
        if (!v->bits8 && !(v->elided && g_cfg.elide_volume >= 2)) {
            if (int r = dev_alloc((void**)&v->bits8, (size_t)v->ny * v->nx8() * v->pitch8() + 64)) return r;
        }
        A.bits8 = v->bits8;
        A.nx8 = v->nx8();
        A.pitch8 = v->pitch8();
        A.iso = iso_hint;
        {
            const unsigned tpb = 512u / (unsigned)kSampleRpw;
            const int force = g_cfg.sample_mode;
            int mode = (v->nz % 256) == 0 ? 0 : 1;
            if (force == 0 && (v->nz & 3) == 0) mode = 0;
            if (force == 1 || v->ny > 65535 || v->nx8() > 65535) mode = 1;
            static const char* const names[2][2] = {{"sdfk_sample_bits", "sdfk_sample_bits_flat"}, {"sdfk_sample_bits_clip", "sdfk_sample_bits_clip_flat"}};
            hipFunction_t fn = nullptr, fn_colors = nullptr;
            const bool two_pass = !v->elided && p->writes_color && v->colors &&
                                  (g_cfg.color_passes == 2 || (g_cfg.color_passes == 0 && p->n_ops <= kTwoPassMaxOps && v->nvox() >= kTwoPassMinVoxels));
            const int pk = v->elided ? (mode ? PK_SIGNS_FLAT : PK_SIGNS)
                         : two_pass ? (clip_to_bounds ? PK_BITS_NC_CLIP : PK_BITS_NC) + mode
                                    : (clip_to_bounds ? PK_BITS_CLIP : PK_BITS) + mode;
            if (!(v->elided && g_cfg.elide_volume >= 2))
                if (int r = program_fn(p, pk, &fn)) return r;
            if (two_pass)
                if (int r = program_fn(p, PK_COLORS, &fn_colors)) return r;
            const bool cull = v->elided && g_cfg.elide_volume >= 2;
            static const char* const names_nc[2][2] = {{"sdfk_sample_bits_nc", "sdfk_sample_bits_nc_flat"}, {"sdfk_sample_bits_nc_clip", "sdfk_sample_bits_nc_clip_flat"}};
            std::unique_ptr<ProfScope> ps(new ProfScope(cull ? nullptr : (v->elided ? (mode ? "sdfk_sample_signs_flat" : "sdfk_sample_signs")
                                                                                      : (two_pass ? names_nc : names)[clip_to_bounds ? 1 : 0][mode])));
            const size_t plane = (size_t)v->ny * v->pitch();
            phase_token_wait(0);
            if (cull) {
                struct { unsigned long long* bits; unsigned* worklist; unsigned* counter; int nbx, nby, nbz; int cpw; unsigned region; } Cargs;
                Cargs.bits = (unsigned long long*)v->bits;
                Cargs.nbx = v->nxw(); Cargs.nby = (v->ny + 3) / 4; Cargs.nbz = (v->nz + 3) / 4;
                const size_t nblocks = (size_t)Cargs.nbx * Cargs.nby * Cargs.nbz;
                constexpr size_t kLists = 64, kHeader = kLists * 32;

                const size_t ncoarse = (size_t)((Cargs.nbx + 1) / 2) * ((Cargs.nby + 1) / 2) * ((Cargs.nbz + 1) / 2);
                static const int cpw_env = [] { const char* e = getenv("SDFK_CULL_CPW"); return e ? atoi(e) : 0; }();
                Cargs.cpw = cpw_env > 0 ? std::min(cpw_env, 4) : (int)std::min<size_t>(4, std::max<size_t>(1, ncoarse / 4096));
                static const bool coarse_off = [] { const char* e = getenv("SDFK_CULL_COARSE"); return e && atoi(e) == 0; }();
                if (coarse_off) Cargs.cpw = -Cargs.cpw;
                const size_t cull_wgs = (ncoarse + (size_t)std::abs(Cargs.cpw) * 4 - 1) / ((size_t)std::abs(Cargs.cpw) * 4);
                Cargs.region = (unsigned)(((cull_wgs + kLists - 1) / kLists) * (size_t)std::abs(Cargs.cpw) * 32);
                if (!v->cull_list) {
                    if (int r = dev_alloc((void**)&v->cull_list, kLists * (size_t)Cargs.region * sizeof(uint32_t) + kLists * (size_t)Cargs.region + 64)) return r;
                }
                if (!v->cull_header) {
                    auto& clean = g.lanes[g.cur_lane].clean_cull_headers;
                    if (!clean.empty()) { v->cull_header = clean.back(); clean.pop_back(); }
                    else {
                        if (int r = dev_alloc((void**)&v->cull_header, kHeader * sizeof(uint32_t))) return r;
                        HIPCHK(hipMemsetAsync(v->cull_header, 0, kHeader * sizeof(uint32_t), g.stream));
                    }
                    v->cull_header_lane = g.cur_lane;
                } else if (!v->cull_header_clean || v->cull_header_lane != g.cur_lane) {
                    HIPCHK(hipMemsetAsync(v->cull_header, 0, kHeader * sizeof(uint32_t), g.stream));
                    v->cull_header_lane = g.cur_lane;
                }
                v->cull_header_clean = false;
                Cargs.counter = v->cull_header; Cargs.worklist = v->cull_list;
                hipFunction_t fn_cull = nullptr, fn_eval = nullptr;
                if (int r = program_fn(p, PK_CULL, &fn_cull)) return r;
                if (int r = program_fn(p, PK_EVAL_BLOCKS, &fn_eval)) return r;
                void* cparams[] = {&A, &Cargs, p->kargs()};
                {
                    ProfScope ps2("sdfk_cull_blocks");
                    HIPCHK(hipModuleLaunchKernel(fn_cull, (unsigned)cull_wgs, 1, 1, 256, 1, 1, 0, g.stream, cparams, nullptr));
                }
                {
                    ProfScope ps2("sdfk_eval_blocks");
                    HIPCHK(hipModuleLaunchKernel(fn_eval, (unsigned)std::min<size_t>((nblocks + 3) / 4, 4096), 1, 1, 256, 1, 1, 0, g.stream, cparams, nullptr));
                }
            } else if (mode == 1) {
                const dim3 fg = flat_grid(plane, v->nx8());
                HIPCHK(hipModuleLaunchKernel(fn, fg.x, fg.y, fg.z, tpb, 1, 1, 0, g.stream, params, nullptr));
            }
            else
                HIPCHK(hipModuleLaunchKernel(fn, (unsigned)((v->nz + 255) / 256), (unsigned)v->ny,
                                             (unsigned)v->nx8(), tpb, 1, 1, 0, g.stream, params, nullptr));
            ps.reset();
            if (two_pass) {
                ProfScope ps2("sdfk_sample_colors");
                const size_t total = (size_t)v->nx * plane;
                HIPCHK(hipModuleLaunchKernel(fn_colors, (unsigned)((total + 255) / 256), 1, 1, 256, 1, 1, 0, g.stream, params, nullptr));
            }
        }
        phase_token_pass(0);
        if (g.sampler_only) {
            v->bits_valid = false;
            return SDFK_OK;
        }
        if (!(v->elided && g_cfg.elide_volume >= 2)) {
            ProfScope ps("k_bits_transpose");
            hipLaunchKernelGGL(k_bits_transpose, transpose_grid(v->nz, v->ny, v->nxw()), dim3(256), 0, g.stream,
                               v->bits8, v->bits, v->nx8(), v->ny, v->nz, v->nxw(), v->pitch8());
            HIPCHK(hipGetLastError());
        }
        v->bits_iso = iso_hint;
        v->bits_valid = true;
        sampled();
        return SDFK_OK;
    }
}


extern "C" int sdfk_sample(const sdfk_program* p, sdfk_volume* v, int32_t clip_to_bounds)
{
    std::lock_guard<std::recursive_mutex> lk(g_mu);
    if (!p || !v) return fail(SDFK_ERR_INVALID, "sdfk_sample: null argument");
    if (int r = require_init()) return r;
    return sample_impl(p, v, clip_to_bounds, 0.0f);
}

extern "C" int sdfk_volume_clip_to_bounds(sdfk_volume* v)
{
    std::lock_guard<std::recursive_mutex> lk(g_mu);
    if (!v) return fail(SDFK_ERR_INVALID, "null volume");
    if (int r = require_init()) return r;
    float d[3], m[3], outside;
    grid_constants(v, d, m, &outside);
    resolve_dependents(v);
    const size_t face = std::max({(size_t)v->ny * v->nz, (size_t)v->nx * v->nz, (size_t)v->nx * v->ny});
    ProfScope ps("k_clip");
    hipLaunchKernelGGL(k_clip, dim3((unsigned)((face + 255) / 256)), dim3(256), 0, g.stream, v->values, v->nx, v->ny, v->nz, v->pitch(), v->z0,
                       v->nz_global, outside);
    if (v->bits && v->bits_valid)
        hipLaunchKernelGGL(k_clip_bits, dim3((unsigned)(((size_t)v->nz * v->ny + 255) / 256)), dim3(256), 0, g.stream, v->bits, v->nx, v->ny,
                           v->nz, v->z0, v->nz_global, v->nxw(), outside > v->bits_iso ? 1 : 0);
    if (v->sampled_by) v->sampled_args.clip = 1;
    HIPCHK(hipGetLastError());
    return SDFK_OK;
}

int eval_points_launch(const sdfk_program* p, const float* points_dev, int64_t n, float* rgbw_dev)
{
    struct { const float* points; float* rgbw; long n; } A{points_dev, rgbw_dev, (long)n};
    hipFunction_t fn = nullptr;
    if (int r = program_fn(p, PK_POINTS, &fn)) return r;
    void* params[] = {&A, p->kargs()};
    ProfScope ps("sdfk_eval_points");
    HIPCHK(hipModuleLaunchKernel(fn, (unsigned)((n + 255) / 256), 1, 1, 256, 1, 1, 0, g.stream, params, nullptr));
    return SDFK_OK;
}

extern "C" int sdfk_eval_points_device(const sdfk_program* p, const void* points3_dev, int64_t n, void* rgbw4_dev)
{
    std::lock_guard<std::recursive_mutex> lk(g_mu);
    if (!p || n < 0 || (n > 0 && (!points3_dev || !rgbw4_dev))) return fail(SDFK_ERR_INVALID, "sdfk_eval_points: null / negative argument");
    if (n >= (int64_t(1) << 31) * 256) return fail(SDFK_ERR_INVALID, "sdfk_eval_points: too many points");
    if (int r = require_init()) return r;
    if (n == 0) return SDFK_OK;
    return eval_points_launch(p, (const float*)points3_dev, n, (float*)rgbw4_dev);
}

extern "C" int sdfk_eval_points(const sdfk_program* p, const float* points3, int64_t n, float* rgbw4)
{
    std::lock_guard<std::recursive_mutex> lk(g_mu);
    if (!p || n < 0 || (n > 0 && (!points3 || !rgbw4))) return fail(SDFK_ERR_INVALID, "sdfk_eval_points: null / negative argument");
    if (n >= (int64_t(1) << 31) * 256) return fail(SDFK_ERR_INVALID, "sdfk_eval_points: too many points");
    if (int r = require_init()) return r;
    if (n == 0) return SDFK_OK;
    Staged st;
    const float* pd = st.in(points3, (size_t)n * 3);
    float* od = p->writes_color ? st.out(rgbw4, (size_t)n * 4) : st.inout(rgbw4, (size_t)n * 4);
    st.run([&] { return eval_points_launch(p, pd, n, od); });
    return st.finish("sdfk_eval_points");
}

int raymarch_launch(const sdfk_program* p, int32_t width, int32_t height, const float cam[3], const float vpi[16],
                           float nearp, float farp, int32_t iters, float* depth_dev, float* rgb_dev)
{
    RayArgs A;
    memset(&A, 0, sizeof A);
    A.depth = depth_dev; A.rgb = rgb_dev;
    memcpy(A.cam, cam, sizeof A.cam);
// ... 44 lines not shown
```

sdfkit_amd/csrc/mc_kernels.h:

```cpp
#pragma once
#include <hip/hip_runtime.h>
#include <stdint.h>

#include "mc_params.h"

namespace sdfk {

#ifndef SDFK_COMPACT_LPB
#define SDFK_COMPACT_LPB 1
#endif
constexpr int K2_LPB = SDFK_COMPACT_LPB;
static_assert(K2_LPB >= 1 && K2_LPB <= 8, "sign planes per workgroup are held in registers");

struct SlabHeader { int64_t nv, ni; float bmin[3], bmax[3]; int32_t vbytes; int32_t cap_v; int32_t idx_bits; int32_t flags; float pad[2]; };
constexpr int SLAB_IDX_BLOCK = 1024;
static_assert(sizeof(SlabHeader) == 64, "SDFK_SLAB_HEADER_BYTES");

struct PackArgs {
    const McCounters* counters;
    uint32_t cap_active, cap_v;
    uint64_t cap_i;
    const float* vertices;
    const float* colors;
    const float* normals;
    const int32_t* triangles;
    const float* bounds;
    char* dst;
    int64_t capacity;
    int vbytes;
};

struct XformArgs {
    float* vertices;
    float* normals;
    int64_t n;
    float m[16], nm[16];
    float* partial;
};

template <bool FLAT> __global__ void k_signbits8(const float* __restrict__ values, uint8_t* __restrict__ bits8, int nx, int ny, int nz, int nx8, int pitch, float iso);
extern template __global__ void k_signbits8<true>(const float* __restrict__ values, uint8_t* __restrict__ bits8, int nx, int ny, int nz, int nx8, int pitch, float iso);
extern template __global__ void k_signbits8<false>(const float* __restrict__ values, uint8_t* __restrict__ bits8, int nx, int ny, int nz, int nx8, int pitch, float iso);
__global__ void k_bits_transpose(const uint8_t* __restrict__ bits8, uint64_t* __restrict__ bits, int nx8, int ny, int nz, int nxw, int pitch8);
template <bool WRITE> __global__ void k_compact(McParams P);
extern template __global__ void k_compact<true>(McParams P);
extern template __global__ void k_compact<false>(McParams P);
template <bool MASKS> __global__ void k_compact_write(McParams P);
extern template __global__ void k_compact_write<true>(McParams P);
extern template __global__ void k_compact_write<false>(McParams P);
__global__ void k_blockscan(McParams P);
__global__ void k_publish(McParams P);
__global__ void k_chunkscan(McParams P);
__global__ void k_gather_corners(McParams P);
__global__ void k_resolve(McParams P);
template <bool ISO0> __global__ void k_vertices(McParams P, McMeshOut M);
extern template __global__ void k_vertices<true>(McParams P, McMeshOut M);
extern template __global__ void k_vertices<false>(McParams P, McMeshOut M);
__global__ void k_spin(int ticks, int* sink);
__global__ void k_triangles(McParams P, McMeshOut M);
__global__ void k_clip(float* __restrict__ values, int nx, int ny, int nz, int pitch, int z0, int nz_global, float outside);
__global__ void k_clip_bits(uint64_t* __restrict__ bits, int nx, int ny, int nz, int z0, int nz_global, int nxw, int bit);
__global__ void k_slab_header(SlabHeader* dst, int64_t nv, int64_t ni, const float* __restrict__ bounds, int vbytes);
__global__ void k_pack_pending(PackArgs A);
__global__ void k_payload_compact(const char* __restrict__ src, char* __restrict__ dst, int64_t dst_capacity, unsigned long long* __restrict__ ticket);
__global__ void k_slabs_rebase(char* __restrict__ gathered, int world, int64_t stride, SlabHeader* mirror, int mirror_only);
__global__ void k_mesh_transform(XformArgs A);
__global__ void k_bounds_reduce(const float* __restrict__ partial, int blocks, float* __restrict__ bounds);
__global__ void k_slabs_decode16(const char* __restrict__ gathered, int world, int64_t stride, SlabHeader* mirror, int32_t* __restrict__ out, int64_t out_capacity);
__global__ void k_subsample(const float* __restrict__ src, const float* __restrict__ srcc, float* __restrict__ dst, float* __restrict__ dstc, int nx, int ny, int sp, int mx, int my, int mz, int dp, int step);
template <bool TO_PITCHED> __global__ void k_repitch(const float* __restrict__ src, float* __restrict__ dst, size_t rows, int w, int pw);
extern template __global__ void k_repitch<true>(const float* __restrict__ src, float* __restrict__ dst, size_t rows, int w, int pw);
extern template __global__ void k_repitch<false>(const float* __restrict__ src, float* __restrict__ dst, size_t rows, int w, int pw);

}
```

sdfkit_amd/csrc/mc_kernels.hip:

```cpp
#include <hip/hip_runtime.h>
#include <limits.h>
#include <stdint.h>
#include "mc_device.h"
#include "mc_kernels.h"

namespace sdfk {

#ifndef SDFK_K4_WMAX
#define SDFK_K4_WMAX 576
#endif
#ifndef SDFK_K4_RMAX
#define SDFK_K4_RMAX 1024
#endif
constexpr int K4_WMAX = SDFK_K4_WMAX;
constexpr int K4_RMAX = SDFK_K4_RMAX;
static_assert(K4_WMAX <= 768 && K4_WMAX > 512, "k_vertices stages the windows in three rounds of 256 slots");
#ifndef SDFK_K5_VMAX
#define SDFK_K5_VMAX 1536
#endif
constexpr int K5_VMAX = SDFK_K5_VMAX;
static_assert(K5_VMAX % 256 == 0 && K5_VMAX >= 256, "k_triangles loads the block in rounds of 256 slots");

template <bool FLAT>
__global__ __launch_bounds__(256) void k_signbits8(const float* __restrict__ values, uint8_t* __restrict__ bits8, int nx, int ny,
                                                   int nz, int nx8, int pitch, float iso)
{
    __shared__ unsigned char nib[8][64];
    const int lane = threadIdx.x & 63, wave = threadIdx.x >> 6;
    const int x8 = FLAT ? (int)(blockIdx.z + blockIdx.y * 65535u) : (int)blockIdx.z;
    if (x8 >= nx8) return;
    int iy = blockIdx.y, z = blockIdx.x * 256 + 4 * lane;
    bool zok = z < pitch;
    if (FLAT) {
        const int f0 = blockIdx.x * 256, iy0 = f0 / pitch;
        iy = iy0;
        z = (f0 - iy0 * pitch) + 4 * lane;
        const int q = z / pitch;
        z -= q * pitch;
        iy += q;
        zok = f0 + 4 * lane < ny * pitch;
    }
    float v[2][4];
#pragma unroll
    for (int rr = 0; rr < 2; rr++) {
        const int ix = x8 * 8 + wave * 2 + rr;
        v[rr][0] = v[rr][1] = v[rr][2] = v[rr][3] = -INFINITY;
        if (ix < nx && zok) {
            const float4 q = *reinterpret_cast<const float4*>(values + ((size_t)ix * ny + iy) * pitch + z);
            v[rr][0] = q.x;
            if (z + 1 < nz) v[rr][1] = q.y;
            if (z + 2 < nz) v[rr][2] = q.z;
            if (z + 3 < nz) v[rr][3] = q.w;
            if (z >= nz) v[rr][0] = -INFINITY;
        }
    }
#pragma unroll
    for (int rr = 0; rr < 2; rr++) {
        const unsigned n = (v[rr][0] > iso ? 1u : 0u) | (v[rr][1] > iso ? 2u : 0u) | (v[rr][2] > iso ? 4u : 0u) | (v[rr][3] > iso ? 8u : 0u);
        nib[wave * 2 + rr][lane] = (unsigned char)n;
    }
    __syncthreads();
    if (wave == 0 && zok) {
        unsigned out = 0;
#pragma unroll
        for (int r = 0; r < 8; r++) {
            const unsigned q = nib[r][lane];
            out |= ((q & 1u) << r) | (((q >> 1) & 1u) << (8 + r)) | (((q >> 2) & 1u) << (16 + r)) | (((q >> 3) & 1u) << (24 + r));
        }
        *reinterpret_cast<unsigned*>(bits8 + ((size_t)iy * nx8 + x8) * pitch + z) = out;
    }
}

__global__ __launch_bounds__(256) void k_bits_transpose(const uint8_t* __restrict__ bits8, uint64_t* __restrict__ bits,
                                                        int nx8, int ny, int nz, int nxw, int pitch8)
{
    __shared__ __attribute__((aligned(4))) uint8_t t[64][132];
    const int ztiles = (nz + 127) / 128;
    const int iy = (int)(blockIdx.x / (unsigned)ztiles), z0 = (int)(blockIdx.x % (unsigned)ztiles) * 128;
    const int xw0 = (int)(blockIdx.z + blockIdx.y * 65535u) * 8, row0 = xw0 * 8;
    if (xw0 >= nxw) return;
    unsigned v[8];
#pragma unroll
    for (int i = 0; i < 8; i++) {
        const int k = (int)threadIdx.x + 256 * i;
        const int row = k >> 5, c = (k & 31) * 4;
        v[i] = 0;
        if (row0 + row < nx8 && z0 + c < nz)
// ... 31 lines not shown
__device__ __forceinline__ uint64_t wave_sum_u64(uint64_t v)
{
#pragma unroll
    for (int o = 32; o > 0; o >>= 1) v += __shfl_xor(v, o);
    return v;
}

__device__ __forceinline__ uint32_t wave_sum_u32(uint32_t v)
{
#pragma unroll
    for (int o = 32; o > 0; o >>= 1) v += __shfl_xor(v, o);
    return v;
}

__device__ __forceinline__ uint32_t block_excl_scan_u32(uint32_t v, uint32_t& red, uint32_t* total)
{
    __shared__ uint32_t s_incl[4], s_red[4];
    const int lane = threadIdx.x & 63, wave = threadIdx.x >> 6;
    uint32_t incl = v;
#pragma unroll
    for (int o = 1; o < 64; o <<= 1) {
        const uint32_t n = __shfl_up(incl, o);
        if (lane >= o) incl += n;
    }
    const uint32_t r = wave_sum_u32(red);
    __syncthreads();
    if (lane == 63) { s_incl[wave] = incl; s_red[wave] = r; }
    __syncthreads();
    uint32_t pre = incl - v;
    for (int w = 0; w < wave; w++) pre += s_incl[w];
    *total = s_incl[0] + s_incl[1] + s_incl[2] + s_incl[3];
    red = s_red[0] + s_red[1] + s_red[2] + s_red[3];
    return pre;
}

__device__ __forceinline__ uint64_t block_excl_scan_u64(uint64_t v, uint64_t* s_wave , uint64_t* total)
{
    const int lane = threadIdx.x & 63, wave = threadIdx.x >> 6;
    const uint64_t incl = wave_incl_scan_u64(v);
    __syncthreads();
    if (lane == 63) s_wave[wave] = incl;
    __syncthreads();
    uint64_t pre = incl - v;
    for (int w = 0; w < wave; w++) pre += s_wave[w];
    *total = s_wave[0] + s_wave[1] + s_wave[2] + s_wave[3];
    return pre;
}

#ifndef SDFK_KV_XCD_GROUP
#define SDFK_KV_XCD_GROUP 16
#endif
#ifndef SDFK_KR_XCD_GROUP
#define SDFK_KR_XCD_GROUP 16
#endif
#ifndef SDFK_KT_XCD_GROUP
#define SDFK_KT_XCD_GROUP 0
#endif
template <uint32_t G>
__device__ __forceinline__ uint32_t first_chunk_of_block()
{
    const uint32_t b = blockIdx.x;
    if (G == 0) return b;
    const uint32_t span = 8u * (G ? G : 1u), whole = (gridDim.x / span) * span;
    if (b >= whole) return b;
    const uint32_t xcd = b & 7u, q = b >> 3;
    return ((q / (G ? G : 1u)) * 8u + xcd) * G + q % (G ? G : 1u);
}

#ifndef SDFK_K2_XCD_GROUP
#define SDFK_K2_XCD_GROUP 16
#endif
__device__ __forceinline__ int compact_block_of_workgroup(int nlay, int bpl)
{
    constexpr int G = SDFK_K2_XCD_GROUP;
    if (G == 0) return (int)blockIdx.x;
    const int v = (int)first_chunk_of_block<(uint32_t)G>();
    const int GG = G ? G : 1, grouped = (nlay / GG) * GG * bpl;
    if (v >= grouped) return v;
    const int run = v / GG, k = v - run * GG;
    const int lg = run / bpl, part = run - lg * bpl;
    return (lg * GG + k) * bpl + part;
}

__device__ __forceinline__ uint64_t shr1_in(uint64_t w, uint64_t next) { return (w >> 1) | (next << 63); }

typedef unsigned long long u64x2u __attribute__((ext_vector_type(2), aligned(8)));

__device__ __forceinline__ void load_words5(const uint64_t* p, uint64_t* w)
{
    const u64x2u lo = *reinterpret_cast<const u64x2u*>(p);
    const u64x2u hi = *reinterpret_cast<const u64x2u*>(p + 2);
    w[0] = lo.x; w[1] = lo.y; w[2] = hi.x; w[3] = hi.y; w[4] = p[4];
}

__device__ __forceinline__ uint64_t segment_mask(uint64_t a, uint64_t an, uint64_t b, uint64_t bn, uint64_t c, uint64_t cn,
                                                 uint64_t d, uint64_t dn, int rem, uint64_t& m13)
{
    const uint64_t as = shr1_in(a, an), bs = shr1_in(b, bn), cs = shr1_in(c, cn), ds = shr1_in(d, dn);
    const uint64_t valid = rem >= 64 ? ~0ull : (rem <= 0 ? 0ull : ((1ull << rem) - 1ull));
    const uint64_t x1 = a ^ as, x3 = a ^ b, x4 = a ^ c, x6 = a ^ ds;
    const uint64_t eq = (a ^ bs) | (a ^ cs) | (a ^ d);
    m13 = (x1 & x3 & x4 & x6) & ~eq & valid;
    return (x1 | x3 | x4 | x6 | eq) & valid;
}


__device__ __noinline__ void publish_compaction_impl(const uint64_t* blockcnt, McCounters* counters, uint32_t* rowstart_end, int gb, int ge, int nlog)
{
    uint64_t ghost = 0, upto_emit_end = 0, all13 = 0, all = 0;
    const int nt = (int)blockDim.x;
    for (int i0 = threadIdx.x; i0 < nlog; i0 += 4 * nt) {
        uint64_t wv[4];
#pragma unroll
        for (int k = 0; k < 4; k++) wv[k] = i0 + k * nt < nlog ? blockcnt[i0 + k * nt] : 0ull;
#pragma unroll
        for (int k = 0; k < 4; k++) {
            const int i = i0 + k * nt;
            const uint64_t c = wv[k] & 0xffffffffull;
            all += c;
            if (i < gb) ghost += c;
            if (i < ge) upto_emit_end += c;
            all13 += wv[k] >> 32;
        }
    }
    __shared__ uint64_t s_sum[4][16];
    ghost = wave_sum_u64(ghost); upto_emit_end = wave_sum_u64(upto_emit_end); all13 = wave_sum_u64(all13); all = wave_sum_u64(all);
    const int lane = threadIdx.x & 63, wave = threadIdx.x >> 6, nw = nt >> 6;
    if (lane == 0) { s_sum[0][wave] = ghost; s_sum[1][wave] = upto_emit_end; s_sum[2][wave] = all13; s_sum[3][wave] = all; }
    __syncthreads();
    if (threadIdx.x == 0) {
        uint64_t t[4] = {0, 0, 0, 0};
        for (int w = 0; w < nw; w++)
            for (int q = 0; q < 4; q++) t[q] += s_sum[q][w];
        const uint32_t nall = (uint32_t)t[3];
        counters->n_active = nall;
        counters->n_ghost_cells = (uint32_t)t[0];
        counters->n_emit_cells = (uint32_t)(t[1] - t[0]);
        counters->n_case13 = (uint32_t)t[2];
        *rowstart_end = nall;
    }
}

__device__ __forceinline__ void publish_compaction(const McParams& P, int nlay, int nlog)
{
    publish_compaction_impl(P.blockcnt, P.counters, P.rowstart + (size_t)nlay * P.ncy, (P.lay_emit_begin - P.lay_count_begin) * P.bpl,
                            (P.lay_emit_end - P.lay_count_begin) * P.bpl, nlog);
}

template <bool WRITE>
__global__ __launch_bounds__(256) void k_compact(McParams P)
{
    const int nlay = P.lay_list_end - P.lay_count_begin;
    const int nlog = nlay * P.bpl;
    const int wg = K2_LPB == 1 ? compact_block_of_workgroup(nlay, P.bpl) : (int)blockIdx.x;
    const int part = wg % P.bpl, lay0 = (wg / P.bpl) * K2_LPB;
    const int nl = min(K2_LPB, nlay - lay0);
    const int b0 = lay0 * P.bpl + part;
    const int nseg = P.ncy * P.nxw;
    const int i0 = part * 1024 + 4 * (int)threadIdx.x;
    const int wave = (int)(threadIdx.x >> 6);
    bool look[K2_LPB];
#pragma unroll
    for (int l = 0; l < K2_LPB; l++) look[l] = l < nl && (!WRITE || P.wavecnt[(b0 + l * P.bpl) * 4 + wave] != 0);
    uint32_t before[K2_LPB];
#pragma unroll
    for (int l = 0; l < K2_LPB; l++) before[l] = 0;
    if (WRITE) {
        for (int i = threadIdx.x; i < b0; i += 1024) {
            const uint32_t c0 = (uint32_t)P.blockcnt[i];
            const uint32_t c1 = i + 256 < b0 ? (uint32_t)P.blockcnt[i + 256] : 0u;
            const uint32_t c2 = i + 512 < b0 ? (uint32_t)P.blockcnt[i + 512] : 0u;
            const uint32_t c3 = i + 768 < b0 ? (uint32_t)P.blockcnt[i + 768] : 0u;
            before[0] += (c0 + c1) + (c2 + c3);
        }
#pragma unroll
        for (int l = 1; l < K2_LPB; l++)
            if (l < nl)
                for (int i = threadIdx.x; i < P.bpl; i += 256) before[l] += (uint32_t)P.blockcnt[b0 + (l - 1) * P.bpl + i];
    }
    int y0 = 0, xw0 = 0;
    if (i0 < nseg) {
        y0 = i0 / P.nxw;
        xw0 = i0 - y0 * P.nxw;
    }
    uint64_t w[K2_LPB + 1][2][5];
    {
// ... 19 lines not shown
        if (l >= nl) continue;
        uint64_t m[4] = {0, 0, 0, 0};
        uint32_t cnt = 0, n13 = 0;
        if (look[l] && i0 < nseg) {
            int xk = xw0;
#pragma unroll
            for (int k = 0; k < 4; k++) {
                const int rem = (i0 + k < nseg) ? P.ncx - xk * 64 : 0;
                uint64_t m13;
                m[k] = segment_mask(w[l][0][k], w[l][0][k + 1], w[l][1][k], w[l][1][k + 1], w[l + 1][0][k], w[l + 1][0][k + 1],
                                    w[l + 1][1][k], w[l + 1][1][k + 1], rem, m13);
                cnt += (uint32_t)__popcll(m[k]);
                n13 += (uint32_t)__popcll(m13);
                if (++xk == P.nxw) xk = 0;
            }
        }
        if (!WRITE) {
            cnts[l] = cnt; n13s[l] = n13;
            if (P.segmask && __builtin_amdgcn_ballot_w64(cnt != 0u) != 0ull) {
                uint64_t* q = P.segmask + ((size_t)(b0 + l * P.bpl) * 1024u + 4u * threadIdx.x);
                *reinterpret_cast<u64x2u*>(q) = u64x2u{m[0], m[1]};
                *reinterpret_cast<u64x2u*>(q + 2) = u64x2u{m[2], m[3]};
            }
            continue;
        }
        uint32_t total, red = before[l];
        const uint32_t pre = block_excl_scan_u32(cnt, red, &total);
        base_acc += red;
        const int lay = lay0 + l, z = P.lay_count_begin + lay;
        if (b0 == 0 && l == 0) {
            publish_compaction(P, nlay, nlog);
        }
        if (i0 < nseg) {
            uint32_t pos = base_acc + pre;
            uint32_t* rowstart = P.rowstart + (size_t)lay * P.ncy;
            int y = y0, xw = xw0;
#pragma unroll
            for (int k = 0; k < 4; k++) {
                if (i0 + k < nseg) {
                    if (xw == 0) rowstart[y] = pos;
                    const uint32_t yz = (uint32_t)y << P.xbits;
                    uint64_t mk = m[k];
                    while (mk) {
                        const int bit = __builtin_ctzll(mk);
                        mk &= mk - 1;
                        if (pos < P.cap_active) {
                            P.rec_xy[pos] = (uint32_t)(xw * 64 + bit) | yz;
                            P.rec_z[pos] = (uint32_t)z;
                        }
                        pos++;
                    }
                    if (++xw == P.nxw) { xw = 0; y++; }
                }
            }
        }
    }
    if (!WRITE) {
        if (P.zero_cull && blockIdx.x == 0 && threadIdx.x < 64) P.zero_cull[32 * threadIdx.x] = 0u;
        __shared__ uint32_t s_cnt[K2_LPB][4], s_n13[K2_LPB];
        if (threadIdx.x < K2_LPB) s_n13[threadIdx.x] = 0;
        uint32_t wsum[K2_LPB];
#pragma unroll
        for (int l = 0; l < K2_LPB; l++) wsum[l] = wave_sum_u32(cnts[l]);
        __syncthreads();
        if ((threadIdx.x & 63) == 0) {
#pragma unroll
            for (int l = 0; l < K2_LPB; l++)
                if (l < nl) {
                    s_cnt[l][wave] = wsum[l];
                    P.wavecnt[(b0 + l * P.bpl) * 4 + wave] = wsum[l];
                }
        }
#pragma unroll
        for (int l = 0; l < K2_LPB; l++)
            if (n13s[l]) atomicAdd(&s_n13[l], n13s[l]);
        __syncthreads();
        if ((int)threadIdx.x < nl) {
            const int l = (int)threadIdx.x;
            P.blockcnt[b0 + l * P.bpl] = (uint64_t)(s_cnt[l][0] + s_cnt[l][1] + s_cnt[l][2] + s_cnt[l][3]) | ((uint64_t)s_n13[l] << 32);
        }
    }
}

#ifndef SDFK_KW_MINWAVES
#define SDFK_KW_MINWAVES 1
#endif
template <bool MASKS>
__global__ __launch_bounds__(256, MASKS ? SDFK_KW_MINWAVES : 1) void k_compact_write(McParams P)
{
    const int nlay = P.lay_list_end - P.lay_count_begin, nlog = nlay * P.bpl;
    const int b = compact_block_of_workgroup(nlay, P.bpl);
    const int lay = b / P.bpl, part = b - lay * P.bpl;
    const int z = P.lay_count_begin + lay;
    const int nseg = P.ncy * P.nxw;
    const int s0 = part * 1024 + (int)threadIdx.x;
    uint32_t before = 0;
    if (P.blockpre) {
        if (threadIdx.x == 0) before = P.blockpre[b];
    } else {
        for (int i = threadIdx.x; i < b; i += 1024) {
            const uint32_t c0 = (uint32_t)P.blockcnt[i];
            const uint32_t c1 = i + 256 < b ? (uint32_t)P.blockcnt[i + 256] : 0u;
            const uint32_t c2 = i + 512 < b ? (uint32_t)P.blockcnt[i + 512] : 0u;
            const uint32_t c3 = i + 768 < b ? (uint32_t)P.blockcnt[i + 768] : 0u;
            before += (c0 + c1) + (c2 + c3);
        }
    }
    bool look[4];
#pragma unroll
    for (int k = 0; k < 4; k++) look[k] = P.wavecnt[b * 4 + k] != 0;
    uint64_t m[4] = {0, 0, 0, 0};
    int ys[4] = {0, 0, 0, 0}, xws[4] = {0, 0, 0, 0};
    if (MASKS) {
        const uint64_t* q = P.segmask + (size_t)b * 1024u + threadIdx.x;
#pragma unroll
        for (int k = 0; k < 4; k++)
            if (look[k] && s0 + 256 * k < nseg) m[k] = q[256 * k];
#pragma unroll
        for (int k = 0; k < 4; k++) {
            const int s = s0 + 256 * k;
            if (s < nseg) { ys[k] = s / P.nxw; xws[k] = s - ys[k] * P.nxw; }
        }
    } else {
        const size_t plane = (size_t)P.ny * P.nxw;
        const uint64_t* f0 = P.bits + (size_t)z * plane;
        u64x2u wa[4], wb[4], wc[4], wd[4];
#pragma unroll
        for (int k = 0; k < 4; k++) {
            const int s = s0 + 256 * k;
            wa[k] = wb[k] = wc[k] = wd[k] = u64x2u{0, 0};
            if (look[k] && s < nseg) {
                const uint64_t* q = f0 + s;
                wa[k] = *reinterpret_cast<const u64x2u*>(q);
                wb[k] = *reinterpret_cast<const u64x2u*>(q + P.nxw);
                wc[k] = *reinterpret_cast<const u64x2u*>(q + plane);
                wd[k] = *reinterpret_cast<const u64x2u*>(q + plane + P.nxw);
            }
        }
#pragma unroll
        for (int k = 0; k < 4; k++) {
            const int s = s0 + 256 * k;
            if (s < nseg) {
                ys[k] = s / P.nxw;
                xws[k] = s - ys[k] * P.nxw;
                if (look[k]) {
                    uint64_t m13;
                    m[k] = segment_mask(wa[k].x, wa[k].y, wb[k].x, wb[k].y, wc[k].x, wc[k].y, wd[k].x, wd[k].y, P.ncx - xws[k] * 64, m13);
                }
            }
        }
    }
    __shared__ uint64_t s_wave[4];
    const uint64_t mine = (uint64_t)__popcll(m[0]) | ((uint64_t)__popcll(m[1]) << 16) | ((uint64_t)__popcll(m[2]) << 32) | ((uint64_t)__popcll(m[3]) << 48);
    uint64_t total;
    const uint64_t pre = block_excl_scan_u64(mine, s_wave, &total);
    __shared__ uint32_t s_before[4];
    {
        const uint32_t r = wave_sum_u32(before);
        if ((threadIdx.x & 63) == 0) s_before[threadIdx.x >> 6] = r;
    }
    __syncthreads();
    const uint32_t base = s_before[0] + s_before[1] + s_before[2] + s_before[3];
    if (b == 0 && !P.blockpre) {
        publish_compaction(P, nlay, nlog);
    }
    uint32_t* rowstart = P.rowstart + (size_t)lay * P.ncy;
    uint32_t qbase = base;
#pragma unroll
    for (int k = 0; k < 4; k++) {
        const int s = s0 + 256 * k;
        if (s < nseg) {
            uint32_t pos = qbase + (uint32_t)((pre >> (16 * k)) & 0xffffull);
            if (xws[k] == 0) rowstart[ys[k]] = pos;
            const uint32_t yz = (uint32_t)ys[k] << P.xbits;
            uint64_t mk = m[k];
            while (mk) {
                const int bit = __builtin_ctzll(mk);
                mk &= mk - 1;
                if (pos < P.cap_active) {
                    P.rec_xy[pos] = (uint32_t)(xws[k] * 64 + bit) | yz;
                    P.rec_z[pos] = (uint32_t)z;
                }
                pos++;
            }
        }
        qbase += (uint32_t)((total >> (16 * k)) & 0xffffull);
    }
}

constexpr int SCAN_PER = 16;
template <class T>
__device__ __forceinline__ T scan_1024(T sum, T* s_w , T* tile_total)
{
    const int lane = threadIdx.x & 63, wave = threadIdx.x >> 6;
    T incl = sum;
#pragma unroll
    for (int o = 1; o < 64; o <<= 1) {
        const T n = __shfl_up(incl, o);
        if (lane >= o) incl += n;
    }
// ... 159 lines not shown
    const CornersLds v{col, 256, (double)iso};
    int index = 0;
#pragma unroll
    for (int k = 0; k < 8; k++) index |= (v[k] > 0.0) ? (1 << k) : 0;
    if (index != 0xA5 && index != 0x5A) return false;
    const Tiling t = mc_resolve(lut, v);
    return t.nt == 0;
}

__constant__ int8_t c_pred[12][3][3] = {
    {{0, -1, -1}, {0, 0, -1}, {0, -1, 0}},
    {{0, 0, -1}, {1, 0, -1}, {9, 9, 9}},
    {{0, 0, -1}, {0, 1, -1}, {9, 9, 9}},
    {{-1, 0, -1}, {0, 0, -1}, {-1, 0, 0}},
    {{0, -1, 0}, {9, 9, 9}, {9, 9, 9}},
    {{9, 9, 9}, {9, 9, 9}, {9, 9, 9}},
    {{9, 9, 9}, {9, 9, 9}, {9, 9, 9}},
    {{-1, 0, 0}, {9, 9, 9}, {9, 9, 9}},
    {{-1, -1, 0}, {0, -1, 0}, {-1, 0, 0}},
    {{0, -1, 0}, {1, -1, 0}, {9, 9, 9}},
    {{9, 9, 9}, {9, 9, 9}, {9, 9, 9}},
    {{-1, 0, 0}, {9, 9, 9}, {9, 9, 9}}};

__device__ __forceinline__ bool edge_has_live_predecessor(const McParams& P, const int8_t* lut, int e, int x, int y,
                                                          int z, bool check_dead, float* col)
{
    for (int k = 0; k < 3; k++) {
        const int dx = c_pred[e][k][0];
        if (dx == 9) break;
        const int px = x + dx, py = y + c_pred[e][k][1], pz = z + c_pred[e][k][2];
        if (px < 0 || py < 0 || px >= P.ncx || py >= P.ncy) continue;
        if (pz < 0) {
            if (P.z0 + pz >= 0) return true;
            continue;
        }
        if (pz >= P.ncz) continue;
        if (!check_dead || !cell_is_dead(lut, P.values, P.ny, P.nzp, P.iso, px, py, pz, col)) return true;
    }
    return false;
}

__device__ __forceinline__ unsigned positional_own_mask(bool X, bool Y, bool Z)
{
    unsigned m = (1u << 5) | (1u << 6) | (1u << 10);
    if (!Y) m |= (1u << 4) | (1u << 9);
    if (!X) m |= (1u << 7) | (1u << 11);
    if (!Z) m |= (1u << 1) | (1u << 2);
    if (!Y && !Z) m |= 1u << 0;
    if (!X && !Z) m |= 1u << 3;
    if (!X && !Y) m |= 1u << 8;
    return m;
}

__global__ __launch_bounds__(256) void k_gather_corners(McParams P)
{
    const uint32_t n = min(P.counters->n_active, P.cap_active);
    const size_t sx = (size_t)P.ny * P.nzp, sy = (size_t)P.nzp;
    for (uint32_t i = blockIdx.x * 256u + threadIdx.x; i < n; i += gridDim.x * 256u) {
        const uint32_t xy = P.rec_xy[i];
        const float* p = P.values + (size_t)(xy & P.xmask) * sx + (size_t)(xy >> P.xbits) * sy + P.rec_z[i];
        const f2u q0 = *reinterpret_cast<const f2u*>(p), q1 = *reinterpret_cast<const f2u*>(p + sx);
        const f2u q3 = *reinterpret_cast<const f2u*>(p + sy), q2 = *reinterpret_cast<const f2u*>(p + sx + sy);
        *reinterpret_cast<float4*>(P.rec_corners + (size_t)i * 8) = make_float4(q0.x, q1.x, q2.x, q3.x);
        *reinterpret_cast<float4*>(P.rec_corners + (size_t)i * 8 + 4) = make_float4(q0.y, q1.y, q2.y, q3.y);
    }
}

__global__ __launch_bounds__(256, 5) void k_resolve(McParams P)
{
    __shared__ float s_v[8 * 256];
    __shared__ __attribute__((aligned(16))) int8_t s_lut[MCDEC_PADDED];
    __shared__ uint64_t s_wave[4];
    __shared__ uint64_t s_ord[MCLUT_NROWS];
    __shared__ uint32_t s_rows[2][2];
    mc_load_dec_to_lds(s_lut);
    {
        const int t = (int)threadIdx.x;
        static_assert(MCLUT_NROWS <= 768, "row table copy assumes <= 3 rounds");
        const uint64_t a0 = c_roword[min(t, MCLUT_NROWS - 1)], a1 = c_roword[min(t + 256, MCLUT_NROWS - 1)];
        const uint64_t a2 = c_roword[min(t + 512, MCLUT_NROWS - 1)];
        if (t < MCLUT_NROWS) s_ord[t] = a0;
        if (t + 256 < MCLUT_NROWS) s_ord[t + 256] = a1;
        if (t + 512 < MCLUT_NROWS) s_ord[t + 512] = a2;
    }
    __syncthreads();
    const uint32_t n = min(P.counters->n_active, P.cap_active);
    const bool any13 = P.counters->n_case13 != 0;
    const bool check_dead = any13 && P.values != nullptr;
    const int nchunks = (int)((n + MC_CHUNK - 1u) / MC_CHUNK);
    float* col = s_v + threadIdx.x;
    int parity = 0;
    for (int c = (int)first_chunk_of_block<SDFK_KR_XCD_GROUP>(); c < nchunks; c += gridDim.x, parity ^= 1) {
        const uint32_t i = (uint32_t)c * MC_CHUNK + threadIdx.x;
        const bool mine_rec = threadIdx.x < MC_CHUNK && i < n;
        uint32_t nown = 0, nt_emit = 0, nslots = 0, info = 0, dead = 0;
        uint64_t own = 0;
        int ry = 0, rz = 0;
        if (mine_rec) {
            const uint32_t xy = P.rec_xy[i];
            const int x = (int)(xy & P.xmask), y = (int)(xy >> P.xbits), z = (int)P.rec_z[i];
            ry = y; rz = z;
            corners_to_column(*reinterpret_cast<const float4*>(P.rec_corners + (size_t)i * 8),
                              *reinterpret_cast<const float4*>(P.rec_corners + (size_t)i * 8 + 4), col);
            const CornersLds v{col, 256, (double)P.iso};
            const Tiling t = mc_resolve(s_lut, v);
            const bool counted = z < P.lay_emit_end;
            const bool emit = counted && z >= P.lay_emit_begin;
            if (t.nt > 0) {
                const uint64_t ord = s_ord[t.row];
                const int nd = (int)(ord >> 60);
                if (counted) {
                    const unsigned pmask = positional_own_mask(x > 0, y > 0, P.z0 + z > 0) | (1u << 12);
                    for (int k = 0; k < nd; k++) {
                        const int e = (int)((ord >> (4 * k)) & 15ull);
                        bool mine = (pmask >> e) & 1u;
                        if (check_dead && !mine)
                            mine = !edge_has_live_predecessor(P, s_lut, e, x, y, z, true, col);
                        if (mine) {
                            own |= (uint64_t)e << (4 * nown);
                            nown++;
                        }
                    }
                }
                nt_emit = emit ? (uint32_t)t.nt : 0u;
                nslots = emit ? (uint32_t)nd : 0u;
                info = (1u << 13) | (nt_emit << 14) | (nown << 18) | ((uint32_t)t.row << 22);
            } else if (emit && (t.index == 0xA5 || t.index == 0x5A)) {
                dead = 1;
            }
        }
        const uint32_t first = (uint32_t)c * MC_CHUNK, last = min(first + MC_CHUNK - 1u, n - 1u);
        if (mine_rec && (i == first || i == last)) {
            const uint32_t row = (uint32_t)(rz - P.lay_count_begin) * (uint32_t)P.ncy + (uint32_t)ry;
            if (i == first) s_rows[parity][0] = row;
            if (i == last) s_rows[parity][1] = row;
        }
        uint64_t total;
        const uint64_t pre = block_excl_scan_u64(((uint64_t)nslots << 42) | ((uint64_t)nown << 21) | nt_emit, s_wave, &total);
        const uint32_t rf = s_rows[parity][0], rl = s_rows[parity][1];
        const uint32_t nrows = (uint32_t)((P.lay_list_end - P.lay_count_begin) * P.ncy);
        const uint32_t nrs = min(rl - rf + 3u, (uint32_t)K4_RMAX);
        uint32_t wrow = 0;
        if (threadIdx.x < 3) {
            const uint32_t r = threadIdx.x == 0 ? rf + nrs - 1u : (threadIdx.x == 1 ? rf + (uint32_t)P.ncy : rf + (uint32_t)P.ncy + nrs - 1u);
            wrow = min(P.rowstart[min(r, nrows)], n);
        }
        if (mine_rec) {
            P.rec_info[i] = info ? info | (uint32_t)(pre >> 42) : 0u;
            P.rec_own[i] = own;
            P.rec_pre[i] = (uint32_t)((pre >> 21) & 0x1fffffull) | ((uint32_t)(pre & 0x1fffffull) << 16);
        }
        uint64_t ndead = 0;
        if (any13) (void)block_excl_scan_u64(dead, s_wave, &ndead);
        const uint32_t w1e = __shfl(wrow, 0), w2s = __shfl(wrow, 1), w2e = __shfl(wrow, 2);
        if (threadIdx.x == 0) {
            P.chunktot[c] = (((total >> 21) & 0x1fffffull) << 31) | (total & 0x1fffffull);
            P.chunkslots[c] = (uint32_t)(total >> 42);
            P.chunkdead[c] = (uint32_t)ndead;
            P.chunkwin[c] = make_uint4(rf, rl, w1e, w2s);
            P.chunkwin2[c] = w2e;
        }
    }
}

__device__ __forceinline__ uint32_t block_exclusive_scan_256(uint32_t v, uint32_t* s_pre , uint32_t* s_wave )
{
// ... 695 lines not shown
    for (int b = threadIdx.x; b < blocks; b += 256) {
#pragma unroll
        for (int j = 0; j < 3; j++) r[j] = fminf(r[j], partial[(size_t)b * 6 + j]);
#pragma unroll
        for (int j = 3; j < 6; j++) r[j] = fmaxf(r[j], partial[(size_t)b * 6 + j]);
    }
#pragma unroll
    for (int o = 32; o > 0; o >>= 1) {
#pragma unroll
        for (int j = 0; j < 3; j++) r[j] = fminf(r[j], __shfl_down(r[j], o));
#pragma unroll
        for (int j = 3; j < 6; j++) r[j] = fmaxf(r[j], __shfl_down(r[j], o));
    }
    const int lane = threadIdx.x & 63, wave = threadIdx.x >> 6;
    if (lane == 0) {
#pragma unroll
        for (int j = 0; j < 6; j++) s_red[j][wave] = r[j];
    }
    __syncthreads();
    if (threadIdx.x < 6) {
        const int j = threadIdx.x;
        float a = s_red[j][0];
        for (int w = 1; w < 4; w++) a = (j < 3) ? fminf(a, s_red[j][w]) : fmaxf(a, s_red[j][w]);
        bounds[j] = a;
    }
}

__global__ __launch_bounds__(256) void k_slabs_decode16(const char* __restrict__ gathered, int world, int64_t stride, SlabHeader* mirror,
                                                        int32_t* __restrict__ out, int64_t out_capacity)
{
    const int r = blockIdx.y;
    if (mirror && blockIdx.x == 0 && threadIdx.x < sizeof(SlabHeader) / 4)
        reinterpret_cast<uint32_t*>(mirror + r)[threadIdx.x] =
            reinterpret_cast<const uint32_t*>(gathered + (size_t)r * stride)[threadIdx.x];
    int64_t vbase = 0, ibase = 0;
    for (int q = 0; q < world; q++) {
        const SlabHeader* hq = reinterpret_cast<const SlabHeader*>(gathered + (size_t)q * stride);
        if (hq->nv < 0 || hq->ni < 0) return;
        if (q < r) { vbase += hq->nv; ibase += hq->ni; }
    }
    const SlabHeader* h = reinterpret_cast<const SlabHeader*>(gathered + (size_t)r * stride);
    if (h->idx_bits != 16 || slab_compact_bytes(h->nv, h->ni, h->vbytes) > stride) return;
    const int64_t ni = h->ni;
    if (ibase + ni > out_capacity) return;
    const char* sec = gathered + (size_t)r * stride + sizeof(SlabHeader) + (int64_t)h->vbytes * h->nv;
    const uint16_t* t16 = reinterpret_cast<const uint16_t*>(sec);
    const int32_t* bases = reinterpret_cast<const int32_t*>(sec + ((2 * ni + 3) & ~int64_t(3)));
    for (int64_t i = (int64_t)blockIdx.x * 256 + threadIdx.x; i < ni; i += (int64_t)gridDim.x * 256)
        out[ibase + i] = bases[i / SLAB_IDX_BLOCK] + (int32_t)t16[i] + (int32_t)vbase;
}

__global__ __launch_bounds__(256) void k_subsample(const float* __restrict__ src, const float* __restrict__ srcc,
                                                   float* __restrict__ dst, float* __restrict__ dstc, int nx, int ny,
                                                   int sp, int mx, int my, int mz, int dp, int step)
{
    const size_t n = (size_t)mx * my * mz;
    for (size_t i = (size_t)blockIdx.x * 256u + threadIdx.x; i < n; i += (size_t)gridDim.x * 256u) {
        const int z = (int)(i % mz);
        const size_t t = i / mz;
        const int y = (int)(t % my);
        const int x = (int)(t / my);
        const size_t o = ((size_t)(x * step) * ny + (size_t)(y * step)) * sp + (size_t)(z * step);
        const size_t d = ((size_t)x * my + y) * dp + z;
        dst[d] = src[o];
        if (srcc) { dstc[d * 3] = srcc[o * 3]; dstc[d * 3 + 1] = srcc[o * 3 + 1]; dstc[d * 3 + 2] = srcc[o * 3 + 2]; }
    }
}

template <bool TO_PITCHED>
__global__ __launch_bounds__(256) void k_repitch(const float* __restrict__ src, float* __restrict__ dst, size_t rows, int w, int pw)
{
    const size_t n = rows * (size_t)w;
    for (size_t i = (size_t)blockIdx.x * 256u + threadIdx.x; i < n; i += (size_t)gridDim.x * 256u) {
        const size_t r = i / w, c = i - r * w;
        if (TO_PITCHED) dst[r * pw + c] = src[i];
        else dst[i] = src[r * pw + c];
    }
}

template __global__ void k_signbits8<true>(const float* __restrict__ values, uint8_t* __restrict__ bits8, int nx, int ny, int nz, int nx8, int pitch, float iso);
template __global__ void k_signbits8<false>(const float* __restrict__ values, uint8_t* __restrict__ bits8, int nx, int ny, int nz, int nx8, int pitch, float iso);
template __global__ void k_compact<true>(McParams P);
template __global__ void k_compact<false>(McParams P);
template __global__ void k_compact_write<true>(McParams P);
template __global__ void k_compact_write<false>(McParams P);
template __global__ void k_vertices<true>(McParams P, McMeshOut M);
template __global__ void k_vertices<false>(McParams P, McMeshOut M);
template __global__ void k_repitch<true>(const float* __restrict__ src, float* __restrict__ dst, size_t rows, int w, int pw);
template __global__ void k_repitch<false>(const float* __restrict__ src, float* __restrict__ dst, size_t rows, int w, int pw);

}
```

sdfkit_amd/csrc/mc_params.h:

```cpp
#pragma once
#include <hip/hip_runtime.h>
#include <stdint.h>

namespace sdfk {

#ifndef MC_CHUNK_RECORDS
#define MC_CHUNK_RECORDS 240
#endif
constexpr uint32_t MC_CHUNK = MC_CHUNK_RECORDS;
static_assert(MC_CHUNK >= 64 && MC_CHUNK <= 256, "one 256-thread workgroup per chunk");
#ifndef SDFK_SCAN_BLOCKS
#define SDFK_SCAN_BLOCKS 8192
#endif
#ifndef SDFK_SCAN_CHUNKS
#define SDFK_SCAN_CHUNKS 8192
#endif
constexpr int MC_SCAN_BLOCKS = SDFK_SCAN_BLOCKS;
constexpr uint32_t MC_SCAN_CHUNKS = SDFK_SCAN_CHUNKS;
constexpr uint32_t MC_VSTRIDE = MC_CHUNK * 13u;
static_assert(MC_VSTRIDE <= 4096, "the in-chunk slot prefix has 12 bits in rec_info");

struct McCounters {
    uint32_t n_active;
    uint32_t n_case13;
    uint32_t n_dead;
    uint32_t total_v;
    uint32_t total_t;
    uint32_t nghost;
    uint32_t n_ghost_cells;
    uint32_t overflow;
    uint32_t n_emit_cells;
    uint32_t pad[7];
};

struct McParams {
    const float* values;
    const float* colors;
    int nx, ny, nz;
    int nzp;
    int ncx, ncy, ncz;
    int nxw;
    int z0;
    int lay_count_begin;
    int lay_emit_begin;
    int lay_emit_end;
    int lay_list_end;
    float iso;
    int step;
    const uint64_t* bits;
    uint32_t* zero_cull;
    int bpl;
    uint64_t* blockcnt;
    uint32_t* wavecnt;
    uint64_t* segmask;
    uint32_t* blockpre;
    uint64_t* chunktot;
    uint64_t* chunkpre;
    int chunkscan;
    uint32_t* rec_xy;
    int xbits;
    uint32_t xmask;
    uint32_t* rec_z;
    uint32_t* rowstart;
    uint32_t* rec_info;
    uint64_t* rec_own;
    uint32_t* rec_pre;
    float* rec_corners;
    uint32_t* rec_vid;
    uint32_t* chunkslots;
    uint32_t* chunkdead;
    uint4* chunkwin;
    uint32_t* chunkwin2;
    uint32_t cap_active;
    McCounters* counters;
    McCounters* host_counters;
};

struct McMeshOut {
    float* vertices;
    float* colors;
    float* normals;
    float* grid_vertices;
    int32_t* triangles;
    uint32_t cap_vertices;
    size_t cap_indices;
    int64_t vertex_base;
    float sc[3], tr[3];
    float inv[3];
    float* bounds_partial;
    int bounds_blocks;
    float* bounds;
    float* host_bounds;
    void* slab_header;
    int32_t slab_vbytes;
    uint2* vdesc;
};

}
```

Baseline: 953,600.

## Count active cells directly from sign bytes, skipping bit transpose

For full-volume step-1 sample-march, the bit-transpose pass and the layered bitword volume are skipped. A new k_count_bytes kernel builds segment masks and per-block counts straight from the byte-packed sign bits, using an in-register 8x8 transpose. It also writes per-segment validity ballots so the strided compact-write kernel only reads masks that were actually written. The count buffers are zeroed inside a later kernel and recycled through a per-lane clean pool, which avoids a memset per call. This adds new paths and eligibility conditions and carries correctness risk at z-chunk edges and in the clean-buffer state tracking.

```diff
diff --git a/include/sdfkit_hip.h b/include/sdfkit_hip.h
--- a/include/sdfkit_hip.h
+++ b/include/sdfkit_hip.h
@@ -75,7 +75,8 @@
     SDFK_OPT_IDLE_PROGRAMS = 15,
     SDFK_OPT_ELIDE_VOLUME = 16,
     SDFK_OPT_COLOR_PASSES = 17,
-    SDFK_OPT_COUNT_ = 18
+    SDFK_OPT_COUNT_BYTES = 18,
+    SDFK_OPT_COUNT_ = 19
 } sdfk_option;
 int sdfk_set_option(int32_t key, int64_t value);
 int sdfk_get_option(int32_t key, int64_t* value);
diff --git a/sdfkit_amd/_native.py b/sdfkit_amd/_native.py
--- a/sdfkit_amd/_native.py
+++ b/sdfkit_amd/_native.py
@@ -195,6 +195,7 @@
 OPT_IDLE_PROGRAMS = 15
 OPT_ELIDE_VOLUME = 16
 OPT_COLOR_PASSES = 17
+OPT_COUNT_BYTES = 18
 
 
 def library_path():
diff --git a/sdfkit_amd/build.py b/sdfkit_amd/build.py
--- a/sdfkit_amd/build.py
+++ b/sdfkit_amd/build.py
@@ -11,7 +11,7 @@
 SOURCES = ["lib_context.hip", "lib_jit.hip", "lib_volume.hip", "lib_march.hip", "lib_mesh.hip", "lib_dist.hip", "mc_kernels.hip", "lib_points.hip",
            "lib_trimesh.hip", "lib_redistance.hip", "lib_points_knn.hip", "lib_pointcloud.hip", "lib_orient.hip", "lib_points_filter.hip", "lib_trimesh_topology.hip",
            "lib_trimesh_smooth.hip", "lib_trimesh_weld.hip", "lib_points_cluster.hip", "lib_trimesh_simplify.hip", "lib_trimesh_ray.hip"]
-HEADERS = ["lib_internal.h", "device_stage.h", "points_grid.h", "points_set.h", "points_knn.h", "points_walk.h", "points_normals.h", "points_orient.h", "points_filter.h", "points_color.h", "points_cluster.h", "device_forest.h", "icp_solve.h", "trimesh_sdf.h", "trimesh_sample.h", "trimesh_handle.h", "trimesh_topology.h", "trimesh_adjacency.h", "trimesh_weld.h", "trimesh_simplify.h", "trimesh_ray.h", "device_sort.h", "redistance.h", "device_scan.h", "device_reduce.h", "mc_kernels.h", "mc_device.h", "mc_decide.h", "mc_params.h", "mc_luts.h", "sample_codegen.h", "vol_pyramid.h", "mathops.h", "dist_rccl.h", "node_local.h",
+HEADERS = ["lib_internal.h", "device_stage.h", "points_grid.h", "points_set.h", "points_knn.h", "points_walk.h", "points_normals.h", "points_orient.h", "points_filter.h", "points_color.h", "points_cluster.h", "device_forest.h", "icp_solve.h", "trimesh_sdf.h", "trimesh_sample.h", "trimesh_handle.h", "trimesh_topology.h", "trimesh_adjacency.h", "trimesh_weld.h", "trimesh_simplify.h", "trimesh_ray.h", "device_sort.h", "redistance.h", "device_scan.h", "device_reduce.h", "mc_kernels.h", "mc_device.h", "mc_decide.h", "mc_signbytes.h", "mc_params.h", "mc_luts.h", "sample_codegen.h", "vol_pyramid.h", "mathops.h", "dist_rccl.h", "node_local.h",
            "slab_protocol.h", os.path.join("..", "..", "include", "sdfkit_hip.h")]
 DEPS = ["exports.map"] + SOURCES + HEADERS
 CFLAGS = ["--offload-arch=gfx950", "-O3", "-std=c++17", "-ffp-contract=off", "-fPIC", "-fno-fast-math", "-fvisibility=hidden", "-Wall",
diff --git a/sdfkit_amd/csrc/lib_context.hip b/sdfkit_amd/csrc/lib_context.hip
--- a/sdfkit_amd/csrc/lib_context.hip
+++ b/sdfkit_amd/csrc/lib_context.hip
@@ -464,6 +464,7 @@
     g_cfg.prefault_huge = geti("SDFK_PREFAULT_HUGE", 0) ? 1 : 0;
     g_cfg.place_streams = geti("SDFK_STREAM_PLACEMENT", 1) ? 1 : 0;
     g_cfg.idle_lane = geti("SDFK_IDLE_LANE", 1) ? 1 : 0;
+    g_cfg.count_bytes = geti("SDFK_COUNT_BYTES", 1) ? 1 : 0;
     g_cfg.sample_mode = geti("SDFK_SAMPLE_MODE", -1);
     g_cfg.hw_queues = geti("GPU_MAX_HW_QUEUES", 0);
     g_cfg.env_cache_dir = gets("SDFK_CACHE_DIR");
@@ -575,6 +576,7 @@
         for (auto& kv : lane.free_blocks) (void)hipFree(kv.second);
         lane.free_blocks.clear();
         lane.clean_cull_headers.clear();
+        lane.clean_counts.clear();
     }
     for (auto& kv : g.live_blocks) (void)hipFree(kv.first);
     g.live_blocks.clear();
@@ -703,6 +705,7 @@
     case SDFK_OPT_DIST_INDEX16: if (!in(0, 1)) break; g_cfg.dist_index16 = (int)value; return SDFK_OK;
     case SDFK_OPT_STREAM_PLACEMENT: if (!in(0, 1)) break; g_cfg.place_streams = (int)value; return SDFK_OK;
     case SDFK_OPT_IDLE_LANE: if (!in(0, 1)) break; g_cfg.idle_lane = (int)value; return SDFK_OK;
+    case SDFK_OPT_COUNT_BYTES: if (!in(0, 1)) break; g_cfg.count_bytes = (int)value; return SDFK_OK;
     case SDFK_OPT_CODE_CACHE: if (!in(0, 1)) break; g_cfg.code_cache = (int)value; return SDFK_OK;
     case SDFK_OPT_IDLE_PROGRAMS: if (!in(0, 1024)) break; g_cfg.idle_programs = (int)value; codes_trim(); return SDFK_OK;
     case SDFK_OPT_ELIDE_VOLUME: if (!in(0, 2)) break; g_cfg.elide_volume = (int)value; return SDFK_OK;
@@ -731,6 +734,7 @@
     case SDFK_OPT_DIST_INDEX16: *value = g_cfg.dist_index16; break;
     case SDFK_OPT_STREAM_PLACEMENT: *value = g_cfg.place_streams; break;
     case SDFK_OPT_IDLE_LANE: *value = g_cfg.idle_lane; break;
+    case SDFK_OPT_COUNT_BYTES: *value = g_cfg.count_bytes; break;
     case SDFK_OPT_CODE_CACHE: *value = g_cfg.code_cache; break;
     case SDFK_OPT_IDLE_PROGRAMS: *value = g_cfg.idle_programs; break;
     case SDFK_OPT_ELIDE_VOLUME: *value = g_cfg.elide_volume; break;
diff --git a/sdfkit_amd/csrc/lib_internal.h b/sdfkit_amd/csrc/lib_internal.h
--- a/sdfkit_amd/csrc/lib_internal.h
+++ b/sdfkit_amd/csrc/lib_internal.h
@@ -56,6 +56,7 @@
     int prefault_huge = 0;
     int place_streams = 1;
     int idle_lane = 1;
+    int count_bytes = 1;
     int copy_threads = 0;
     int sample_mode = -1;
     int hw_queues = 0;
@@ -89,7 +90,8 @@
     hipStream_t user_stream = nullptr;
     hipStream_t own_stream = nullptr;
     static constexpr int NSIDE = 4;
-    struct Lane { hipStream_t stream = nullptr; std::multimap<size_t, void*> free_blocks; std::vector<uint32_t*> clean_cull_headers; };
+    struct Lane { hipStream_t stream = nullptr; std::multimap<size_t, void*> free_blocks; std::vector<uint32_t*> clean_cull_headers;
+                  std::multimap<size_t, void*> clean_counts; };
     Lane lanes[1 + NSIDE];
     struct Placed { hipStream_t s; int cls; int user; };
     std::vector<Placed> pool;
@@ -358,6 +360,7 @@
     uint8_t* bits8 = nullptr;
     float bits_iso = 0.0f;
     bool bits_valid = false;
+    bool bytes_only = false;
     sdfk_program* sampled_by = nullptr;
     SampleArgs sampled_args;
     int pitch() const { return (nz + 3) & ~3; }
@@ -411,6 +414,10 @@
     bool finished = false;
     bool empty = false;
     bool have_bits = false;
+    bool count_bytes = false;
+    void* counts = nullptr;
+    size_t counts_bytes = 0;
+    bool counts_clean = false;
     uint8_t* bits8 = nullptr;
     sdfk_program* eval_prog = nullptr;
     SampleArgs eval_args;
diff --git a/sdfkit_amd/csrc/lib_march.hip b/sdfkit_amd/csrc/lib_march.hip
--- a/sdfkit_amd/csrc/lib_march.hip
+++ b/sdfkit_amd/csrc/lib_march.hip
@@ -52,6 +52,11 @@
     }
     for (void* p : j->owned) dev_free(p);
     j->owned.clear();
+    if (j->counts) {
+        if (j->counts_clean && g.lanes[j->lane].clean_counts.size() < 16) g.lanes[j->lane].clean_counts.emplace(j->counts_bytes, j->counts);
+        else dev_free(j->counts);
+        j->counts = nullptr;
+    }
     if (j->eval_prog) program_release(j->eval_prog);
     j->eval_prog = nullptr;
     if (j->sub) {
@@ -117,13 +122,18 @@
     {
         ProfScope ps("k_compact");
         const int nwg = ((P.lay_list_end - P.lay_count_begin + K2_LPB - 1) / K2_LPB) * P.bpl;
-        hipLaunchKernelGGL(k_compact<false>, dim3(nwg), dim3(256), 0, g.stream, P);
+        if (j->count_bytes) {
+            j->counts_clean = false;
+            hipLaunchKernelGGL(k_count_bytes, dim3((unsigned)(P.ncy + 3) / 4, (unsigned)P.nxw, (unsigned)(P.ncz + 511) / 512), dim3(256), 0, g.stream, P);
+        } else
+            hipLaunchKernelGGL(k_compact<false>, dim3(nwg), dim3(256), 0, g.stream, P);
         HIPCHK(hipGetLastError());
         if (P.zero_cull && j->cull_clean && nwg > 0) *j->cull_clean = true;
         if (P.blockpre) hipLaunchKernelGGL(k_blockscan, dim3(1), dim3(1024), 0, g.stream, P);
         if (SDFK_COMPACT_STRIDED && K2_LPB == 1)
-            if (P.segmask) hipLaunchKernelGGL(k_compact_write<true>, dim3((P.lay_list_end - P.lay_count_begin) * P.bpl), dim3(256), 0, g.stream, P);
-            else hipLaunchKernelGGL(k_compact_write<false>, dim3((P.lay_list_end - P.lay_count_begin) * P.bpl), dim3(256), 0, g.stream, P);
+            if (j->count_bytes) hipLaunchKernelGGL((k_compact_write<true, true>), dim3((P.lay_list_end - P.lay_count_begin) * P.bpl), dim3(256), 0, g.stream, P);
+            else if (P.segmask) hipLaunchKernelGGL((k_compact_write<true, false>), dim3((P.lay_list_end - P.lay_count_begin) * P.bpl), dim3(256), 0, g.stream, P);
+            else hipLaunchKernelGGL((k_compact_write<false, false>), dim3((P.lay_list_end - P.lay_count_begin) * P.bpl), dim3(256), 0, g.stream, P);
         else
             hipLaunchKernelGGL(k_compact<true>, dim3(nwg), dim3(256), 0, g.stream, P);
         HIPCHK(hipGetLastError());
@@ -149,6 +159,7 @@
         if (P.chunkscan) hipLaunchKernelGGL(k_chunkscan, dim3(1), dim3(1024), 0, g.stream, P);
         if (publish) hipLaunchKernelGGL(k_publish, dim3(1), dim3(256), 0, g.stream, P);
         HIPCHK(hipGetLastError());
+        j->counts_clean = true;
     }
     return SDFK_OK;
 }
@@ -242,16 +253,38 @@
         j->eval_prog->refs++;
         j->eval_args = v->sampled_args;
     }
-    j->have_bits = (step == 1 && v->bits && v->bits_valid && v->bits_iso == iso);
-    if (j->have_bits) P.bits = v->bits;
+    const int nlog = (P.lay_list_end - P.lay_count_begin) * P.bpl;
+    j->count_bytes = step == 1 && v->bytes_only && v->bits8 && v->bits_valid && v->bits_iso == iso && !slab && P.lay_count_begin == 0 &&
+                     P.lay_list_end == P.ncz && nlog <= MC_SCAN_BLOCKS && SDFK_COMPACT_STRIDED && K2_LPB == 1 && SDFK_COMPACT_MASKS;
+    j->have_bits = j->count_bytes || (step == 1 && v->bits && v->bits_valid && v->bits_iso == iso);
+    if (j->count_bytes) {
+        P.bits = nullptr;
+        P.bits8 = v->bits8; P.nx8 = v->nx8(); P.pitch8 = v->pitch8();
+        P.nsegp = (P.ncy * P.nxw + 7) & ~7;
+        r = r ? r : job_alloc(j, &P.segvalid, (size_t)((P.ncz + 511) / 512) * 8 * P.nsegp);
+    } else if (j->have_bits) P.bits = v->bits;
     else {
         uint64_t* bits = nullptr;
         r = r ? r : job_alloc(j, &bits, (size_t)P.nz * P.ny * P.nxw + 8);
         P.bits = bits;
         r = r ? r : job_alloc(j, &j->bits8, (size_t)P.ny * ((P.nx + 7) / 8) * ((P.nz + 3) & ~3) + 64);
     }
-    r = r ? r : job_alloc(j, &P.blockcnt, (size_t)(P.lay_list_end - P.lay_count_begin) * P.bpl + 1);
-    r = r ? r : job_alloc(j, &P.wavecnt, (size_t)(P.lay_list_end - P.lay_count_begin) * P.bpl * 4 + 4);
+    if (j->count_bytes && !r) {
+        j->counts_bytes = ((size_t)nlog + 1) * sizeof(uint64_t) + ((size_t)nlog * 4 + 4) * sizeof(uint32_t);
+        auto& clean = g.lanes[g.cur_lane].clean_counts;
+        auto it = clean.find(j->counts_bytes);
+        if (it != clean.end()) { j->counts = it->second; clean.erase(it); }
+        else {
+            r = dev_alloc(&j->counts, j->counts_bytes);
+            if (!r && hipMemsetAsync(j->counts, 0, j->counts_bytes, g.stream) != hipSuccess) r = fail(SDFK_ERR_HIP, "hipMemsetAsync failed");
+        }
+        j->counts_clean = !r;
+        P.blockcnt = (uint64_t*)j->counts;
+        P.wavecnt = (uint32_t*)((char*)j->counts + ((size_t)nlog + 1) * sizeof(uint64_t));
+    } else {
+        r = r ? r : job_alloc(j, &P.blockcnt, (size_t)nlog + 1);
+        r = r ? r : job_alloc(j, &P.wavecnt, (size_t)nlog * 4 + 4);
+    }
     P.segmask = nullptr;
     if (SDFK_COMPACT_STRIDED && K2_LPB == 1 && SDFK_COMPACT_MASKS)
         r = r ? r : job_alloc(j, &P.segmask, (size_t)(P.lay_list_end - P.lay_count_begin) * P.bpl * 1024 + 4);
@@ -1131,6 +1164,15 @@
     return r;
 }
 
+static bool count_bytes_applies(const sdfk_volume* v, int step)
+{
+    if (!g_cfg.count_bytes || step != 1 || v->z0 != 0 || v->nz != v->nz_global || v->nx < 2 || v->ny < 2 || v->nz < 2) return false;
+    if (v->elided && g_cfg.elide_volume >= 2) return false;
+    if ((v->pitch8() & 7) != 0 || v->nxw() > 65535) return false;
+    const size_t bpl = ((size_t)(v->ny - 1) * v->nxw() + 1023) / 1024;
+    return bpl * (size_t)(v->nz - 1) <= (size_t)MC_SCAN_BLOCKS && SDFK_COMPACT_STRIDED && K2_LPB == 1 && SDFK_COMPACT_MASKS;
+}
+
 extern "C" int sdfk_sample_march(const sdfk_program* p, const float min[3], const float max[3],
                                  int32_t nx, int32_t ny, int32_t nz, int32_t clip_to_bounds,
                                  float iso_value, int32_t step, sdfk_mesh** out)
@@ -1172,6 +1214,7 @@
         const int dflt = (int64_t)nx * ny * nz >= (int64_t(1) << 27) ? 1 : 0;
         g.token_mask = (lane > 0 && g.side_lanes > 1) ? (g_cfg.tokens >= 0 ? g_cfg.tokens : dflt) : 0;
     }
+    if (!r) v->bytes_only = count_bytes_applies(v, step);
     if (!r) r = sample_impl(p, v, clip_to_bounds, step == 1 ? iso_value : 0.0f);
     if (!r) r = sdfk_march(v, iso_value, step, out);
     g.token_mask = 0;
diff --git a/sdfkit_amd/csrc/lib_volume.hip b/sdfkit_amd/csrc/lib_volume.hip
--- a/sdfkit_amd/csrc/lib_volume.hip
+++ b/sdfkit_amd/csrc/lib_volume.hip
@@ -222,7 +222,7 @@
     };
     void* params[] = {&A, p->kargs()};
     {
-        if (!v->bits) {
+        if (!v->bits && !v->bytes_only) {
             if (int r = dev_alloc((void**)&v->bits, v->nbitwords() * sizeof(uint64_t))) return r;
         }
         if (!v->bits8 && !(v->elided && g_cfg.elide_volume >= 2)) {
@@ -317,7 +317,7 @@
             v->bits_valid = false;
             return SDFK_OK;
         }
-        if (!(v->elided && g_cfg.elide_volume >= 2)) {
+        if (!(v->elided && g_cfg.elide_volume >= 2) && !v->bytes_only) {
             ProfScope ps("k_bits_transpose");
             hipLaunchKernelGGL(k_bits_transpose, transpose_grid(v->nz, v->ny, v->nxw()), dim3(256), 0, g.stream,
                                v->bits8, v->bits, v->nx8(), v->ny, v->nz, v->nxw(), v->pitch8());
diff --git a/sdfkit_amd/csrc/mc_kernels.h b/sdfkit_amd/csrc/mc_kernels.h
--- a/sdfkit_amd/csrc/mc_kernels.h
+++ b/sdfkit_amd/csrc/mc_kernels.h
@@ -45,9 +45,11 @@
 template <bool WRITE> __global__ void k_compact(McParams P);
 extern template __global__ void k_compact<true>(McParams P);
 extern template __global__ void k_compact<false>(McParams P);
-template <bool MASKS> __global__ void k_compact_write(McParams P);
-extern template __global__ void k_compact_write<true>(McParams P);
-extern template __global__ void k_compact_write<false>(McParams P);
+__global__ void k_count_bytes(McParams P);
+template <bool MASKS, bool VALID> __global__ void k_compact_write(McParams P);
+extern template __global__ void k_compact_write<true, false>(McParams P);
+extern template __global__ void k_compact_write<false, false>(McParams P);
+extern template __global__ void k_compact_write<true, true>(McParams P);
 __global__ void k_blockscan(McParams P);
 __global__ void k_publish(McParams P);
 __global__ void k_chunkscan(McParams P);
diff --git a/sdfkit_amd/csrc/mc_kernels.hip b/sdfkit_amd/csrc/mc_kernels.hip
--- a/sdfkit_amd/csrc/mc_kernels.hip
+++ b/sdfkit_amd/csrc/mc_kernels.hip
@@ -3,6 +3,7 @@
 #include <stdint.h>
 #include "mc_device.h"
 #include "mc_kernels.h"
+#include "mc_signbytes.h"
 
 namespace sdfk {
 
@@ -200,7 +201,6 @@
     return (lg * GG + k) * bpl + part;
 }
 
-__device__ __forceinline__ uint64_t shr1_in(uint64_t w, uint64_t next) { return (w >> 1) | (next << 63); }
 
 typedef unsigned long long u64x2u __attribute__((ext_vector_type(2), aligned(8)));
 
@@ -209,17 +209,6 @@
     const u64x2u lo = *reinterpret_cast<const u64x2u*>(p);
     const u64x2u hi = *reinterpret_cast<const u64x2u*>(p + 2);
     w[0] = lo.x; w[1] = lo.y; w[2] = hi.x; w[3] = hi.y; w[4] = p[4];
-}
-
-__device__ __forceinline__ uint64_t segment_mask(uint64_t a, uint64_t an, uint64_t b, uint64_t bn, uint64_t c, uint64_t cn,
-                                                 uint64_t d, uint64_t dn, int rem, uint64_t& m13)
-{
-    const uint64_t as = shr1_in(a, an), bs = shr1_in(b, bn), cs = shr1_in(c, cn), ds = shr1_in(d, dn);
-    const uint64_t valid = rem >= 64 ? ~0ull : (rem <= 0 ? 0ull : ((1ull << rem) - 1ull));
-    const uint64_t x1 = a ^ as, x3 = a ^ b, x4 = a ^ c, x6 = a ^ ds;
-    const uint64_t eq = (a ^ bs) | (a ^ cs) | (a ^ d);
-    m13 = (x1 & x3 & x4 & x6) & ~eq & valid;
-    return (x1 | x3 | x4 | x6 | eq) & valid;
 }
 
 
@@ -405,10 +394,86 @@
     }
 }
 
+__global__ __launch_bounds__(256) void k_count_bytes(McParams P)
+{
+    __shared__ uint32_t s_cnt[512], s_n13[512];
+    const int lane = (int)(threadIdx.x & 63), wave = (int)(threadIdx.x >> 6);
+    const int y = (int)blockIdx.x * 4 + wave, xw = (int)blockIdx.y, zc = (int)blockIdx.z * 512;
+    const int nlay = P.lay_list_end;
+    const bool row_ok = y < P.ncy;
+    const int z = zc + 8 * lane;
+    s_cnt[threadIdx.x] = s_cnt[threadIdx.x + 256] = 0;
+    s_n13[threadIdx.x] = s_n13[threadIdx.x + 256] = 0;
+    uint64_t rows[2][9];
+    uint32_t edge[2] = {0, 0};
+#pragma unroll
+    for (int v = 0; v < 2; v++) {
+#pragma unroll
+        for (int t = 0; t < 9; t++) {
+            const int x8 = 8 * xw + t;
+            rows[v][t] = 0;
+            if (row_ok && x8 < P.nx8 && z < P.pitch8)
+                rows[v][t] = *reinterpret_cast<const uint64_t*>(P.bits8 + ((size_t)(y + v) * P.nx8 + x8) * P.pitch8 + z);
+        }
+        if (row_ok && lane < 9 && 8 * xw + lane < P.nx8 && zc + 512 < P.nz)
+            edge[v] = P.bits8[((size_t)(y + v) * P.nx8 + 8 * xw + lane) * P.pitch8 + zc + 512];
+    }
+    if (P.zero_cull && blockIdx.x == 0 && blockIdx.y == 0 && blockIdx.z == 0 && threadIdx.x < 64) P.zero_cull[32 * threadIdx.x] = 0u;
+    __syncthreads();
+    uint64_t w8[2], n8[2];
+#pragma unroll
+    for (int v = 0; v < 2; v++) {
+        uint64_t mine = 0, ew = 0;
+#pragma unroll
+        for (int t = 0; t < 8; t++) {
+            mine |= (rows[v][t] & 0xffull) << (8 * t);
+            ew |= (uint64_t)(__builtin_amdgcn_readlane((int)edge[v], t) & 0xff) << (8 * t);
+        }
+        const uint32_t en = (uint32_t)__builtin_amdgcn_readlane((int)edge[v], 8) & 1u;
+        w8[v] = __shfl_down(mine, 1);
+        n8[v] = (uint64_t)__shfl_down((uint32_t)(rows[v][8] & 1ull), 1);
+        if (lane == 63) { w8[v] = ew; n8[v] = en; }
+    }
+    uint64_t m[8], m13[8];
+    signbytes_lane_masks(rows, w8, n8, P.ncx - xw * 64, row_ok ? nlay - z : 0, m, m13);
+    const int i = y * P.nxw + xw;
+    const int q = i >> 8, q0 = ((int)blockIdx.x * 4 * P.nxw + xw) >> 8;
+    uint64_t ballots = 0;
+#pragma unroll
+    for (int j = 0; j < 8; j++) {
+        const uint64_t bal = __builtin_amdgcn_ballot_w64(m[j] != 0ull);
+        if (lane == j) ballots = bal;
+        if (m[j] != 0ull) {
+            const int lay = z + j;
+            P.segmask[((size_t)lay * P.bpl + (i >> 10)) * 1024u + (unsigned)(i & 1023)] = m[j];
+            const uint32_t c = (uint32_t)__popcll(m[j]), c13 = (uint32_t)__popcll(m13[j]);
+            if (q == q0) {
+                atomicAdd(&s_cnt[8 * lane + j], c);
+                if (c13) atomicAdd(&s_n13[8 * lane + j], c13);
+            } else {
+                atomicAdd(&P.wavecnt[(size_t)lay * P.bpl * 4 + q], c);
+                atomicAdd(reinterpret_cast<unsigned long long*>(&P.blockcnt[(size_t)lay * P.bpl + (q >> 2)]), (unsigned long long)c | ((unsigned long long)c13 << 32));
+            }
+        }
+    }
+    if (row_ok && lane < 8) P.segvalid[((size_t)blockIdx.z * 8 + lane) * P.nsegp + i] = ballots;
+    __syncthreads();
+#pragma unroll
+    for (int k = 0; k < 2; k++) {
+        const int l = (int)threadIdx.x + 256 * k;
+        const uint32_t c = s_cnt[l], c13 = s_n13[l];
+        if (c) {
+            const int lay = zc + l;
+            atomicAdd(&P.wavecnt[(size_t)lay * P.bpl * 4 + q0], c);
+            atomicAdd(reinterpret_cast<unsigned long long*>(&P.blockcnt[(size_t)lay * P.bpl + (q0 >> 2)]), (unsigned long long)c | ((unsigned long long)c13 << 32));
+        }
+    }
+}
+
 #ifndef SDFK_KW_MINWAVES
 #define SDFK_KW_MINWAVES 1
 #endif
-template <bool MASKS>
+template <bool MASKS, bool VALID>
 __global__ __launch_bounds__(256, MASKS ? SDFK_KW_MINWAVES : 1) void k_compact_write(McParams P)
 {
     const int nlay = P.lay_list_end - P.lay_count_begin, nlog = nlay * P.bpl;
@@ -438,7 +503,13 @@
         const uint64_t* q = P.segmask + (size_t)b * 1024u + threadIdx.x;
 #pragma unroll
         for (int k = 0; k < 4; k++)
-            if (look[k] && s0 + 256 * k < nseg) m[k] = q[256 * k];
+            if (look[k] && s0 + 256 * k < nseg) {
+                if (VALID) {
+                    const uint64_t vb = P.segvalid[((size_t)(lay >> 9) * 8 + (lay & 7)) * P.nsegp + s0 + 256 * k];
+                    if ((vb >> ((lay & 511) >> 3)) & 1ull) m[k] = q[256 * k];
+                } else
+                    m[k] = q[256 * k];
+            }
 #pragma unroll
         for (int k = 0; k < 4; k++) {
             const int s = s0 + 256 * k;
@@ -764,6 +835,13 @@
         if (t < MCLUT_NROWS) s_ord[t] = a0;
         if (t + 256 < MCLUT_NROWS) s_ord[t + 256] = a1;
         if (t + 512 < MCLUT_NROWS) s_ord[t + 512] = a2;
+    }
+    {
+        const int nclr = (P.lay_list_end - P.lay_count_begin) * P.bpl * 4 + 4;
+        for (int i = (int)(blockIdx.x * 256u + threadIdx.x); i < nclr; i += (int)(gridDim.x * 256u)) {
+            P.wavecnt[i] = 0u;
+            if (4 * i < nclr) P.blockcnt[i] = 0ull;
+        }
     }
     __syncthreads();
     const uint32_t n = min(P.counters->n_active, P.cap_active);
@@ -1625,8 +1703,9 @@
 template __global__ void k_signbits8<false>(const float* __restrict__ values, uint8_t* __restrict__ bits8, int nx, int ny, int nz, int nx8, int pitch, float iso);
 template __global__ void k_compact<true>(McParams P);
 template __global__ void k_compact<false>(McParams P);
-template __global__ void k_compact_write<true>(McParams P);
-template __global__ void k_compact_write<false>(McParams P);
+template __global__ void k_compact_write<true, false>(McParams P);
+template __global__ void k_compact_write<false, false>(McParams P);
+template __global__ void k_compact_write<true, true>(McParams P);
 template __global__ void k_vertices<true>(McParams P, McMeshOut M);
 template __global__ void k_vertices<false>(McParams P, McMeshOut M);
 template __global__ void k_repitch<true>(const float* __restrict__ src, float* __restrict__ dst, size_t rows, int w, int pw);
diff --git a/sdfkit_amd/csrc/mc_params.h b/sdfkit_amd/csrc/mc_params.h
--- a/sdfkit_amd/csrc/mc_params.h
+++ b/sdfkit_amd/csrc/mc_params.h
@@ -53,6 +53,10 @@
     uint64_t* blockcnt;
     uint32_t* wavecnt;
     uint64_t* segmask;
+    const uint8_t* bits8;
+    int nx8, pitch8;
+    uint64_t* segvalid;
+    int nsegp;
     uint32_t* blockpre;
     uint64_t* chunktot;
     uint64_t* chunkpre;
diff --git a/sdfkit_amd/csrc/mc_signbytes.h b/sdfkit_amd/csrc/mc_signbytes.h
--- /dev/null
+++ b/sdfkit_amd/csrc/mc_signbytes.h
@@ -0,0 +1,61 @@
+#pragma once
+#include <stdint.h>
+
+namespace sdfk {
+
+__device__ __forceinline__ uint64_t shr1_in(uint64_t w, uint64_t next) { return (w >> 1) | (next << 63); }
+
+__device__ __forceinline__ uint64_t segment_mask(uint64_t a, uint64_t an, uint64_t b, uint64_t bn, uint64_t c, uint64_t cn,
+                                                 uint64_t d, uint64_t dn, int rem, uint64_t& m13)
+{
+    const uint64_t as = shr1_in(a, an), bs = shr1_in(b, bn), cs = shr1_in(c, cn), ds = shr1_in(d, dn);
+    const uint64_t valid = rem >= 64 ? ~0ull : (rem <= 0 ? 0ull : ((1ull << rem) - 1ull));
+    const uint64_t x1 = a ^ as, x3 = a ^ b, x4 = a ^ c, x6 = a ^ ds;
+    const uint64_t eq = (a ^ bs) | (a ^ cs) | (a ^ d);
+    m13 = (x1 & x3 & x4 & x6) & ~eq & valid;
+    return (x1 | x3 | x4 | x6 | eq) & valid;
+}
+
+__device__ __forceinline__ void signbytes_transpose8(uint64_t r[8])
+{
+#pragma unroll
+    for (int i = 0; i < 4; i++) {
+        const uint64_t t = ((r[i] >> 32) ^ r[i + 4]) & 0x00000000ffffffffull;
+        r[i + 4] ^= t;
+        r[i] ^= t << 32;
+    }
+#pragma unroll
+    for (int h = 0; h < 8; h += 4)
+#pragma unroll
+        for (int i = h; i < h + 2; i++) {
+            const uint64_t t = ((r[i] >> 16) ^ r[i + 2]) & 0x0000ffff0000ffffull;
+            r[i + 2] ^= t;
+            r[i] ^= t << 16;
+        }
+#pragma unroll
+    for (int i = 0; i < 8; i += 2) {
+        const uint64_t t = ((r[i] >> 8) ^ r[i + 1]) & 0x00ff00ff00ff00ffull;
+        r[i + 1] ^= t;
+        r[i] ^= t << 8;
+    }
+}
+
+__device__ __forceinline__ uint64_t signbytes_next(uint64_t following_row, int j) { return (following_row >> (8 * j)) & 1ull; }
+
+__device__ __forceinline__ void signbytes_lane_masks(uint64_t rows[2][9], const uint64_t w8[2], const uint64_t n8[2], int rem, int nlayers,
+                                                     uint64_t m[8], uint64_t m13[8])
+{
+    signbytes_transpose8(rows[0]);
+    signbytes_transpose8(rows[1]);
+#pragma unroll
+    for (int j = 0; j < 8; j++) {
+        const uint64_t c = j < 7 ? rows[0][j < 7 ? j + 1 : 0] : w8[0], cn = j < 7 ? signbytes_next(rows[0][8], j + 1) : n8[0];
+        const uint64_t d = j < 7 ? rows[1][j < 7 ? j + 1 : 0] : w8[1], dn = j < 7 ? signbytes_next(rows[1][8], j + 1) : n8[1];
+        uint64_t q13;
+        const uint64_t q = segment_mask(rows[0][j], signbytes_next(rows[0][8], j), rows[1][j], signbytes_next(rows[1][8], j), c, cn, d, dn, rem, q13);
+        m[j] = j < nlayers ? q : 0ull;
+        m13[j] = j < nlayers ? q13 : 0ull;
+    }
+}
+
+}
```

Result: faster. 980,800 (median of 6 runs) (+2.9%).
